# fx-erick/uncertainty-vit

Hardware: AMD Instinct MI355X
Metric: pretrain images/sec (ViT-B/16 224, bs=128/GPU) (higher is better)
Workload: dtype bf16

## Files before the change

### include/uvit.h

```cpp
#ifndef UVIT_H
#define UVIT_H
#include <stddef.h>
#include <stdint.h>

#ifdef __cplusplus
extern "C" {
#endif

#define UVIT_VERSION 100
#define UVIT_MAX_DEPTH 64

typedef struct uvit_engine uvit_engine;
typedef void* uvit_stream;

typedef struct uvit_config {
    int32_t img_size, patch_size, in_chans, embed_dim, depth, num_heads, mlp_hidden;
    int32_t use_shared_rel_pos_bias;
    int32_t use_abs_pos_emb;
    int32_t batch;
    float ln_eps;
    float attn_drop_rate;
    float drop_path_rate;
    int32_t bias_chunk;
    int32_t two_stream;
// ... 75 lines not shown
int uvit_step_backward_layer(uvit_engine* e, int layer, const uvit_step_params* hp, uvit_stream stream);
int uvit_step_wait_layer_grads(uvit_engine* e, int layer, uvit_stream stream);
int uvit_step_backward_embed(uvit_engine* e, uvit_stream stream);
int uvit_step_update(uvit_engine* e, const uvit_step_params* hp, uvit_stream stream);
int uvit_train_step(uvit_engine* e, const float* images, const int64_t* mask, const uvit_step_params* hp,
                    uvit_stream stream);
typedef struct uvit_tuning { int32_t nt_variant, tn_variant, tn_split_target, wgrad_group_chunks, nt_group, nt_persist; } uvit_tuning;
void uvit_tuning_default(uvit_tuning* out);
int uvit_engine_set_tuning(uvit_engine* e, const uvit_tuning* t);
int uvit_engine_set_streams(uvit_engine* e, int dual);
int uvit_engine_set_drop_path_rows(uvit_engine* e, int on);
int uvit_drop_path_kept_counts(int depth, float drop_path_rate, int draws_per_block, int batch, uint32_t seed, uint32_t it, int32_t* out);
int uvit_engine_profile(uvit_engine* e, int enable, int max_launches);
int uvit_engine_profile_read(uvit_engine* e, double* total_ms, int* launches, double* flops_per_launch);
int uvit_engine_profile_read_kind(uvit_engine* e, int kind, double* total_ms, int* launches, double* flops_per_launch,
                                  double* bytes_per_launch);
int uvit_engine_read_stats_async(uvit_engine* e, float* host_out2, uvit_stream stream);
int uvit_engine_read_stats(uvit_engine* e, float* host_out2, uvit_stream stream);

typedef struct uvit_gemm_epilogue {
    void* out; void* out2; const float* bias; const float* bias2; const float* gamma; const float* resid;
    const float* rowscale; const void* aux; const int64_t* mask; const float* mask_token;
    int32_t ldo, tokens, patches;
    int32_t row0;
} uvit_gemm_epilogue;
enum { UVIT_EPI_BF16 = 0, UVIT_EPI_QKV = 1, UVIT_EPI_GELU = 2, UVIT_EPI_RESID = 3, UVIT_EPI_F32 = 4,
       UVIT_EPI_PATCH = 5, UVIT_EPI_DGELU = 6, UVIT_EPI_QKV_ELU = 7,
       UVIT_EPI_GELU_DG = 8,
       UVIT_EPI_MULAUX = 9 };

int uvit_op_gemm_nt(int mode, const void* A_bf16, const void* W_bf16, int M, int N, int K, int lda, int ldw,
                    const uvit_gemm_epilogue* epi, uvit_stream stream);
int uvit_op_gemm_nt_tuned(int mode, const void* A_bf16, const void* W_bf16, int M, int N, int K, int lda, int ldw,
                          const uvit_gemm_epilogue* epi, const uvit_tuning* tune, int* tail_rows, uvit_stream stream);
typedef struct uvit_gemm_nt_plan_info { int32_t kernel, rows, grid, tail_rows; } uvit_gemm_nt_plan_info;
int uvit_op_gemm_nt_plan(int mode, int M, int N, int K, int lda, int ldw, int ldo, int row_list,
                         const uvit_tuning* tuning, int num_cu, uvit_gemm_nt_plan_info* out);
int uvit_op_gemm_nt_sched(int mode, const void* A_bf16, const void* W_bf16, int M, int N, int K, int lda, int ldw,
                          const uvit_gemm_epilogue* epi, const uvit_tuning* tune, uint32_t* tile_counters, uvit_stream stream);
int uvit_op_gemm_tn(const void* Y_bf16, const void* X_bf16, int M, int N, int K, int ldy, int ldx, float* C, int ldc,
                    const uvit_tuning* tune, uvit_stream stream);
typedef struct uvit_wgrad_problem {
    const void* Y_bf16; const void* X_bf16; float* C; float* bias; float* bias2;
    int32_t bias_end, bias2_begin, M, N, K, ldy, ldx, ldc;
} uvit_wgrad_problem;
int uvit_op_wgrad_group(const uvit_wgrad_problem* problems, int count, const uvit_tuning* tune, uvit_stream stream);
int uvit_op_attn_fwd(const void* qkv, const float* biasP, void* out, float* lse, int B, int H, int N, int NP,
                     float scale, float p_drop, uint32_t seed, uint32_t layer, uvit_stream stream);
int64_t uvit_op_attn_bwd_ws_bytes(int B, int H, int N);
int uvit_op_attn_bwd(const void* qkv, const void* o_fwd, const void* d_o, const float* biasP, const float* lse,
                           float* delta, void* dqkv, float* dbias_slab, int accumulate_slab, void* ds_workspace, int B, int H,
                           int N, int NP, float scale, float p_drop, uint32_t seed, uint32_t layer, uvit_stream stream);
int uvit_op_attn_fwd_hd(const void* qkv, const float* biasP, void* out, float* lse, int B, int H, int N, int NP, int head_dim,
                        float scale, float p_drop, uint32_t seed, uint32_t layer, uvit_stream stream);
int uvit_op_attn_bwd_hd(const void* qkv, const void* o_fwd, const void* d_o, const float* biasP, const float* lse,
                        float* delta, void* dqkv, float* dbias_slab, int accumulate_slab, void* ds_workspace, int B, int H,
                        int N, int NP, int head_dim, float scale, float p_drop, uint32_t seed, uint32_t layer, uvit_stream stream);
int uvit_op_attn2_fwd(const void* qkv_m, const void* qkv_c, const float* biasP, void* out_m, void* out_c, float* lse, int B, int H,
                      int N, int NP, float scale, float p_drop, uint32_t seed, uint32_t layer, uvit_stream stream);
int64_t uvit_op_attn2_bwd_ws_bytes(int B, int H, int N);
int uvit_op_attn2_bwd(const void* qkv_m, const void* qkv_c, const void* o_m, const void* o_c, const void* d_m, const void* d_c,
                      const float* biasP, const float* lse, float* delta, void* dqkv_m, void* dqkv_c, float* dbias_slab,
                      int accumulate_slab, void* ds_workspace, int B, int H, int N, int NP, float scale, float p_drop, uint32_t seed,
                      uint32_t layer, uvit_stream stream);
int uvit_op_relpos_gather(const float* table, const int32_t* index, float* biasP, int H, int N, int NP, uvit_stream stream);
int uvit_op_relpos_scatter(const float* slab, int nslab, const int32_t* index, float* dtable, int H, int N, int NP,
                           uvit_stream stream);
int uvit_op_ln_fwd(const float* x, const float* w, const float* b, void* y_bf16, float* mean, float* rstd, int M, int C,
                   float eps, uvit_stream stream);
int uvit_op_ln_bwd(const void* dy_bf16, const float* x, const float* mean, const float* rstd, const float* w,
                   const float* dres, float* dx, float* dw, float* db, int M, int C, uvit_stream stream);
int uvit_op_ln_fwd_walk(const float* x, const float* w, const float* b, void* y_bf16, float* mean, float* rstd, int M, int C,
                        float eps, const int32_t* rowidx, const int32_t* count, const int32_t* pos, float* xcopy, int tokens,
                        uvit_stream stream);
typedef struct uvit_ls_rider {
    const void* y; const float* gamma; const float* rowscale; void* dy; float* dgamma; float* dbias;
    int32_t tokens; const int32_t* pos; const int32_t* cnt; int32_t pad_base; void* pad2; int32_t pad2_cols;
} uvit_ls_rider;
int uvit_op_ln_bwd_walk(const void* dy_bf16, const float* x, const float* mean, const float* rstd, const float* w, const float* dres,
                        float* dx, float* dw, float* db, int M, int C, int nrep, int64_t rep_stride, const int32_t* rowidx,
                        const int32_t* count, const int32_t* pos, const uvit_ls_rider* next, uvit_stream stream);
int uvit_op_ls_bwd(const float* dx, const uvit_ls_rider* rider, int M, int C, int nrep, int64_t rep_stride, const int32_t* rowidx,
                   const int32_t* count, uvit_stream stream);
int uvit_op_colsum(const void* y_bf16, int ld, int col0, int ncols, int M, float* out, int nrep, int64_t rep_stride, uvit_stream stream);
int uvit_op_reduce_replicas(const float* rep, float* out, int64_t n, int nrep, int64_t stride, uvit_stream stream);
int uvit_op_droppath_lists(const float* scales, int32_t* pos, int32_t* bmap, int32_t* rows, int32_t* cnt, int nlists, int B, int tokens,
                           int rows_stride, const int32_t* host_counts, uvit_stream stream);
int uvit_op_gemm_nt_rows(int mode, const void* A_bf16, const void* W_bf16, int M, int N, int K, int lda, int ldw,
                         const uvit_gemm_epilogue* epi, const int32_t* rowmap, const int32_t* rowcount, const uvit_tuning* tune,
                         uvit_stream stream);
typedef struct uvit_wgrad_split { float* bias_s1; float* bias2_s1; int32_t s1_row; } uvit_wgrad_split;
int uvit_op_wgrad_group_split(const uvit_wgrad_problem* problems, const uvit_wgrad_split* split, int count, const uvit_tuning* tune,
                              uvit_stream stream);
int uvit_op_token_bwd(const float* dx, const int64_t* mask, void* dpatch_bf16, float* dcls, float* dmask_token, int B, int P, int C,
                      uvit_stream stream);
typedef struct uvit_transpose_desc { const void* src; void* dst; int32_t rows, cols, tile0, pad; } uvit_transpose_desc;
int uvit_op_transpose_batch(const uvit_transpose_desc* descs_dev, int ndesc, int total_tiles, uvit_stream stream);
int uvit_op_ema(float* ema, const float* params, void* ema_bf16, int64_t n, float decay, uvit_stream stream);
int uvit_op_sumsq(const float* g, int64_t n, double* out, uvit_stream stream);
int uvit_op_adamw(float* p, const float* g, float* m, float* v, void* p_bf16, int64_t n, int64_t n_decay, float lr,
                  float wd, float b1, float b2, float eps, int step, const double* sumsq, float max_norm,
                  float grad_scale, float* gnorm_out, uvit_stream stream);
int uvit_op_smooth_l1(const float* out, const float* target, const int32_t* count_dev, float beta, int l2,
                      float loss_scale, float* loss, void* dout_bf16, int Mmax, int C, uvit_stream stream);
int uvit_op_wasserstein_loss(const float* out_m, const float* out_c, const float* tgt_m, const float* tgt_c,
                             const int32_t* count_dev, float lam, float loss_scale, float* scratch, float* loss,
                             void* dout_m_bf16, void* dout_c_bf16, int Mmax, int C, uvit_stream stream);
int uvit_op_target_accum(const float* x, const int32_t* rowidx, const int32_t* count, float* acc, int first, int Mmax,
                         int C, float eps, uvit_stream stream);
int uvit_op_variance_loss(const float* out, const int32_t* count_dev, float w, float margin, float loss_scale, float* scratch,
                          float* loss, float* std_loss0_out, void* dout_bf16, int Mmax, int C, uvit_stream stream);
int uvit_op_target_finalize(float* acc, const int32_t* count, int n_layers, int post_ln, int Mmax, int C, float eps,
                            uvit_stream stream);
int uvit_op_mask_compact(const int64_t* mask, int32_t* rowidx, int32_t* count, int B, int P, uvit_stream stream);
int uvit_op_synth_batch(float* images, int64_t* mask, int B, int chans, int img_size, int patches, int n_mask, uint32_t seed,
                        uint32_t it, uvit_stream stream);
int uvit_op_im2col(const float* img, void* cols_bf16, int B, int Cin, int img_size, int patch, uvit_stream stream);
int uvit_op_droppath(float* scales, const float* rates_dev, int depth, int B, uint32_t seed, uint32_t step,
                     uvit_stream stream);
int uvit_op_cast_bf16(const float* src, void* dst_bf16, int64_t n, uvit_stream stream);

#define UVIT_AUG_LANCZOS 1
#define UVIT_AUG_BILINEAR 2
#define UVIT_AUG_BICUBIC 3
#define UVIT_AUG_HAMMING 5
#define UVIT_AUG_BRIGHTNESS 0
#define UVIT_AUG_CONTRAST 1
#define UVIT_AUG_SATURATION 2
typedef struct uvit_augment_desc {
    int64_t offset;
    int32_t h, w;
    int32_t flip;
    int32_t crop_x, crop_y, crop_w, crop_h;
    int32_t resize_w, resize_h;
    int32_t win_x, win_y;
    int32_t filter;
    int32_t n_jitter;
    int32_t jitter_op[3];
    float jitter_factor[3];
    int32_t reserved;
} uvit_augment_desc;
int64_t uvit_op_augment_ws_bytes(const uvit_augment_desc* desc, int B, int S);
int uvit_op_augment_batch(const uint8_t* pixels, int64_t pixel_bytes, const uvit_augment_desc* desc, int B, int S, const float* mean,
                          const float* std, float* out, void* workspace, int64_t ws_bytes, uvit_stream stream);

int64_t uvit_op_probe_pool_ws_bytes(int B, int N, int C);
int uvit_op_probe_pool_norm(const float* x, float* feat, float* scratch, int B, int N, int C, float eps, uvit_stream stream);
int uvit_op_probe_logits(const float* feat, const float* W, const float* bias, float* logits, int B, int K, int C, uvit_stream stream);
int uvit_op_probe_ce(const float* logits, const int64_t* labels, float smoothing, float* dlogits, float* row_loss, float* loss_out,
                     int32_t* top1_top5, int B, int K, uvit_stream stream);
int uvit_op_probe_head_grad(const float* dlogits, const float* feat, float* dW, float* dbias, int B, int K, int C, uvit_stream stream);

int uvit_op_calib_softmax(const float* logits, float* probs, int B, int K, uvit_stream stream);
int uvit_op_calib_confidence(const float* probs, const int64_t* labels, const double* bounds, int n_bins, int positional_acc, float* row_conf,
                             int32_t* row_pred_correct, double* row_nll, double* bin_table, double* ece_nll, int B, int K,
                             uvit_stream stream);
int uvit_op_calib_tace(const float* probs, const int64_t* labels, double threshold, int n_bins, int positional_acc, double* per_class,
                       double* tace, int B, int K, uvit_stream stream);
int uvit_op_calib_auroc(const float* probs, const int64_t* labels, int32_t* rows, double* out, int B, int K, uvit_stream stream);

int uvit_op_stability_ranks(const float* logits, int32_t* ranks, int R, int K, uvit_stream stream);
int uvit_op_stability_sequences(const int32_t* ranks, double* seq, int V, int F, int K, int noise, uvit_stream stream);

int uvit_op_gp_features(const float* feat, const float* gamma, const float* beta, const float* W_rf, const float* b_rf, float scale,
                        float ln_eps, float* ghat, float* u, float* phi, int B, int C, int D, uvit_stream stream);
int uvit_op_gp_precision_update(const float* phi, float* P, int B, int D, double momentum, uvit_stream stream);
// ... 82 lines not shown
```

### uncertainty-vit_amd/csrc/elementwise.hip

```cpp
#include "common.h"
#include "uvit_internal.h"
#include "rowwise.h"

__global__ void im2col_kernel(const float* __restrict__ img, bf16* __restrict__ cols, int B, int Cin, int S, int p) {
    const int g = S / p, P = g * g, K = Cin * p * p, kc_per_row = K / 8;
    const size_t total = (size_t)B * P * kc_per_row;
    for (size_t idx = blockIdx.x * (size_t)blockDim.x + threadIdx.x; idx < total; idx += (size_t)gridDim.x * blockDim.x) {
        const int kc = idx % kc_per_row;
        const size_t row = idx / kc_per_row;
        const int b = row / P, pp = row % P, py = pp / g, px = pp % g;
        const int k = kc * 8, c = k / (p * p), i = (k % (p * p)) / p, j = k % p;
        const float* src = img + (((size_t)b * Cin + c) * S + py * p + i) * S + px * p + j;
        const float4 a = *(const float4*)src, d = *(const float4*)(src + 4);
        bf16x8 o = {f2bf(a.x), f2bf(a.y), f2bf(a.z), f2bf(a.w), f2bf(d.x), f2bf(d.y), f2bf(d.z), f2bf(d.w)};
        *(bf16x8*)(cols + row * K + k) = o;
    }
}

__global__ __launch_bounds__(1024)
void mask_compact_kernel(const int64_t* __restrict__ mask, int* __restrict__ rowidx, int* __restrict__ count, int B, int P) {
    __shared__ int s_w[16];
    const int n = B * P, tid = threadIdx.x, lane = tid & 63, wave = tid >> 6;
    int base = 0;
    for (int sc = 0; sc < n; sc += 32 * 1024) {
        unsigned bits = 0;
#pragma unroll
        for (int k = 0; k < 32; ++k) {
            const int i = sc + k * 1024 + tid;
            if (i < n && mask[i] != 0) bits |= 1u << k;
        }
        for (int k = 0; k < 32 && sc + k * 1024 < n; ++k) {
            const bool keep = (bits >> k) & 1u;
            const unsigned long long bal = __ballot(keep);
            if (lane == 0) s_w[wave] = __popcll(bal);
            __syncthreads();
            int before = base, tot = 0;
#pragma unroll
            for (int q = 0; q < 16; ++q) { const int v = s_w[q]; tot += v; if (q < wave) before += v; }
            if (keep) {
                const int i = sc + k * 1024 + tid, b = i / P;
                rowidx[before + __popcll(bal & ((1ull << lane) - 1ull))] = b * (P + 1) + 1 + (i - b * P);
            }
            base += tot;
            __syncthreads();
        }
    }
    if (tid == 0) *count = base;
    for (int i = base + tid; i < n; i += 1024) rowidx[i] = 0;
}

__global__ void set_cls_kernel(float* __restrict__ x, const float* __restrict__ cls, int B, int N, int C) {
    const int i = blockIdx.x * blockDim.x + threadIdx.x;
    if (i < B * C) { const int b = i / C, c = i - b * C; x[(size_t)b * N * C + c] = cls[c]; }
}

__global__ void relpos_gather_kernel(const float* __restrict__ table, const int* __restrict__ index,
                                     float* __restrict__ biasP, int H, int N, int NP) {
    const size_t total = (size_t)H * NP * NP;
    for (size_t i = blockIdx.x * (size_t)blockDim.x + threadIdx.x; i < total; i += (size_t)gridDim.x * blockDim.x) {
        const int k = i % NP, q = (i / NP) % NP, h = i / ((size_t)NP * NP);
        float v = 0.f;
        if (k >= N) v = -1e30f;
        else if (q < N && table) v = table[(size_t)index[q * N + k] * H + h] * 1.4426950408889634f;
        biasP[i] = v;
    }
}

__global__ void relpos_scatter_kernel(const float* __restrict__ slab, int nslab, const int* __restrict__ index,
                                      float* __restrict__ dtable, int H, int N, int NP, int ntable) {
    extern __shared__ float tsum[];
    const int h = blockIdx.x;
    for (int i = threadIdx.x; i < ntable; i += blockDim.x) tsum[i] = 0.f;
    __syncthreads();
    const int total = N * N;
    for (int i = blockIdx.y * blockDim.x + threadIdx.x; i < total; i += gridDim.y * blockDim.x) {
        const int k = i / N, q = i - k * N;
        float s = 0.f;
        for (int sl = 0; sl < nslab; ++sl) s += slab[(((size_t)sl * H + h) * NP + k) * NP + q];
        atomicAdd(&tsum[index[q * N + k]], s);
    }
    __syncthreads();
    for (int i = threadIdx.x; i < ntable; i += blockDim.x)
        if (tsum[i] != 0.f) atomicAdd(dtable + (size_t)i * H + h, tsum[i]);
}

#define CP_ROWS 32

template <int NV, int WAVES = 4>
__device__ __forceinline__ void block_col_atomic(float4 (&acc)[NV], float* out, int nv, float (*red)[64 * 4]) {
    const int lane = threadIdx.x & 63, wave = threadIdx.x >> 6;
#pragma unroll
    for (int k = 0; k < NV; ++k) {
        if (64 * k < nv) {
            __syncthreads();
            ((float4*)red[wave])[lane] = acc[k];
            __syncthreads();
            if (wave == 0) {
                float4 s = ((float4*)red[0])[lane];
#pragma unroll
                for (int q = 1; q < WAVES; ++q) { const float4 a = ((float4*)red[q])[lane]; s.x += a.x; s.y += a.y; s.z += a.z; s.w += a.w; }
                const int i = lane + 64 * k;
                if (i < nv) { atomicAdd(out + 4 * i, s.x); atomicAdd(out + 4 * i + 1, s.y); atomicAdd(out + 4 * i + 2, s.z); atomicAdd(out + 4 * i + 3, s.w); }
            }
        }
    }
}

template <int NV>
__global__ __launch_bounds__(256)
void ls_bwd_kernel(const float* __restrict__ dx, const bf16* __restrict__ y, const float* __restrict__ gamma,
                   const float* __restrict__ rowscale, bf16* __restrict__ dy, float* __restrict__ dgamma,
                   float* __restrict__ dbias, int M, int C, int tokens, int nrep, size_t rep_stride,
                   const int* __restrict__ rowidx, const int* __restrict__ count) {
    __shared__ float red[4][64 * 4];
    dgamma += (size_t)(blockIdx.x % nrep) * rep_stride; dbias += (size_t)(blockIdx.x % nrep) * rep_stride;
    const int lane = threadIdx.x & 63, wave = threadIdx.x >> 6, nv = C >> 2;
    float4 ag[NV], ab[NV];
#pragma unroll
    for (int k = 0; k < NV; ++k) { ag[k] = make_float4(0.f, 0.f, 0.f, 0.f); ab[k] = ag[k]; }
    const int row_end = min((int)(blockIdx.x + 1) * CP_ROWS, M);
    const int n_valid = rowidx ? min(*count, M) : M;
    for (int row = blockIdx.x * CP_ROWS + wave; row < row_end; row += 4) {
        if (row >= n_valid) { store_zero_row<NV>(dy + (size_t)row * C, nv, lane); continue; }
        const int xr = rowidx ? rowidx[row] : row;
        const float dp = rowscale ? rowscale[xr / tokens] : 1.0f;
#pragma unroll
        for (int k = 0; k < NV; ++k) {
            const int i = lane + 64 * k;
            if (i < nv) {
                const float4 d = ((const float4*)(dx + (size_t)xr * C))[i];
                const float4 g = ((const float4*)gamma)[i];
                const bf16x4 yy = ((const bf16x4*)(y + (size_t)xr * C))[i];
                ls_apply(d, dp, yy, g, (bf16x4*)(dy + (size_t)row * C) + i, ag[k], ab[k]);
            }
        }
    }
    block_col_atomic(ag, dgamma, nv, red);
    block_col_atomic(ab, dbias, nv, red);
}

#define CS_ROWS 256
__global__ __launch_bounds__(256)
void colsum_kernel(const bf16* __restrict__ y, int ld, int col0, int ncols, int M, float* __restrict__ out, int nrep, size_t rep_stride) {
    __shared__ float red[4][64 * 8];
    out += (size_t)(blockIdx.y % nrep) * rep_stride;
    const int lane = threadIdx.x & 63, wave = threadIdx.x >> 6;
    const int c = blockIdx.x * 512 + lane * 8;
    float acc[8];
#pragma unroll
    for (int j = 0; j < 8; ++j) acc[j] = 0.f;
    const int row_end = min((int)(blockIdx.y + 1) * CS_ROWS, M);
    if (c < ncols) {
        const bf16* base = y + col0 + c;
        int row = blockIdx.y * CS_ROWS + wave;
        for (; row + 12 < row_end; row += 16) {
            const bf16x8 v0 = *(const bf16x8*)(base + (size_t)row * ld), v1 = *(const bf16x8*)(base + (size_t)(row + 4) * ld);
            const bf16x8 v2 = *(const bf16x8*)(base + (size_t)(row + 8) * ld), v3 = *(const bf16x8*)(base + (size_t)(row + 12) * ld);
#pragma unroll
            for (int j = 0; j < 8; ++j) acc[j] += (bf2f(v0[j]) + bf2f(v1[j])) + (bf2f(v2[j]) + bf2f(v3[j]));
        }
        for (; row < row_end; row += 4) {
            const bf16x8 v = *(const bf16x8*)(base + (size_t)row * ld);
#pragma unroll
            for (int j = 0; j < 8; ++j) acc[j] += bf2f(v[j]);
        }
    }
#pragma unroll
    for (int j = 0; j < 8; ++j) red[wave][lane * 8 + j] = acc[j];
    __syncthreads();
    for (int i = threadIdx.x; i < 512; i += 256) {
        const int cc = blockIdx.x * 512 + i;
        if (cc < ncols) atomicAdd(out + cc, red[0][i] + red[1][i] + red[2][i] + red[3][i]);
    }
}

__global__ __launch_bounds__(256)
void smooth_l1_kernel(const float* __restrict__ out, const float* __restrict__ target, const int* __restrict__ count,
                      float beta, int l2, float loss_scale, float* __restrict__ loss, bf16* __restrict__ dout,
                      int Mmax, int C) {
    __shared__ float red[4];
    const int n_valid = min(*count, Mmax);
    const size_t nv = (size_t)Mmax * C / 4, valid = (size_t)n_valid * C / 4;
    const float inv = loss_scale / ((float)n_valid * (float)C);
    float part = 0.f;
    for (size_t i = blockIdx.x * (size_t)blockDim.x + threadIdx.x; i < nv; i += (size_t)gridDim.x * blockDim.x) {
        bf16x4 g = bf16x4_zero();
        if (i < valid) {
            const float4 o = ((const float4*)out)[i], t = ((const float4*)target)[i];
            const float d[4] = {o.x - t.x, o.y - t.y, o.z - t.z, o.w - t.w};
#pragma unroll
            for (int j = 0; j < 4; ++j) {
                const float a = fabsf(d[j]);
                float l, gr;
                if (l2) { l = d[j] * d[j]; gr = 2.0f * d[j]; }
                else if (a < beta) { l = 0.5f * d[j] * d[j] / beta; gr = d[j] / beta; }
                else { l = a - 0.5f * beta; gr = d[j] > 0.f ? 1.0f : (d[j] < 0.f ? -1.0f : 0.f); }
                part += l;
                g[j] = f2bf(gr * inv);
            }
        }
        ((bf16x4*)dout)[i] = g;
    }
    part = wave_sum(part);
    if ((threadIdx.x & 63) == 0) red[threadIdx.x >> 6] = part;
    __syncthreads();
    if (threadIdx.x == 0) atomicAdd(loss, (red[0] + red[1] + red[2] + red[3]) * inv);
}

template <int NV, int TKB_WAVES>
__global__ __launch_bounds__(TKB_WAVES * 64)
void token_bwd_kernel(const float* __restrict__ dx, const int64_t* __restrict__ mask, bf16* __restrict__ dpatch,
                      float* __restrict__ dcls, float* __restrict__ dmask, int B, int P, int C, int rows_per_block) {
    __shared__ float red[TKB_WAVES][64 * 4];
    const int lane = threadIdx.x & 63, wave = threadIdx.x >> 6, nv = C >> 2, N = P + 1;
    float4 ac[NV], am[NV];
#pragma unroll
    for (int k = 0; k < NV; ++k) { ac[k] = make_float4(0.f, 0.f, 0.f, 0.f); am[k] = ac[k]; }
    const int M = B * N;
    const int row_end = min((int)(blockIdx.x + 1) * rows_per_block, M);
    for (int row = blockIdx.x * rows_per_block + wave; row < row_end; row += TKB_WAVES) {
        const int b = row / N, t = row - b * N;
// ... 72 lines not shown
        v = uvit_hash32((uint32_t)b ^ key) >= uvit_drop_threshold(r) ? 1.0f / (1.0f - r) : 0.f;
    }
    scales[i] = v;
}

#define DP_MAX_LISTS 128
struct DpHostCounts { int k[DP_MAX_LISTS]; };
#define DPL_CHUNKS 8
__global__ __launch_bounds__(256)
void droppath_lists_kernel(const float* __restrict__ scales, int* __restrict__ pos, int* __restrict__ bmap, int* __restrict__ rows,
                           int* __restrict__ cnt, int B, int tokens, int rows_stride, DpHostCounts host) {
    extern __shared__ int s_m[];
    const int lb = blockIdx.x;
    const float* sc = scales + (size_t)lb * B;
    int* p = pos + (size_t)lb * B; int* m = bmap + (size_t)lb * B; int* r = rows + (size_t)lb * rows_stride;
    const bool pub = blockIdx.y == 0;
    __shared__ int s_w[4];
    const int lane = threadIdx.x & 63, wave = threadIdx.x >> 6;
    int base = 0;
    for (int b0 = 0; b0 < B; b0 += 256) {
        const int b = b0 + threadIdx.x;
        const bool keep = b < B && sc[b] != 0.f;
        const unsigned long long bal = __ballot(keep);
        if (lane == 0) s_w[wave] = __popcll(bal);
        __syncthreads();
        int before = base;
        for (int q = 0; q < wave; ++q) before += s_w[q];
        const int slot = before + __popcll(bal & ((1ull << lane) - 1ull));
        if (pub && b < B) p[b] = keep ? slot : -1;
        if (keep) { s_m[slot] = b; if (pub) m[slot] = b; }
        base += s_w[0] + s_w[1] + s_w[2] + s_w[3];
        __syncthreads();
    }
    if (pub) {
        for (int b = base + threadIdx.x; b < B; b += 256) m[b] = 0;
        if (threadIdx.x == 0) {
            cnt[lb] = base * tokens;
            cnt[gridDim.x + lb] = base != host.k[lb];
        }
    }
    const int n = base * tokens, npad = (n + 63) & ~63;
    const int per = (npad + DPL_CHUNKS - 1) / DPL_CHUNKS, lo = blockIdx.y * per, hi = min(lo + per, npad);
    for (int i = lo + threadIdx.x; i < hi; i += blockDim.x) {
        const int slot = i / tokens;
        r[i] = i < n ? s_m[slot] * tokens + (i - slot * tokens) : -1;
    }
}

static inline int grid_for(size_t n, int block, int cap = 256 * 8) {
    size_t g = (n + block - 1) / block;
    return (int)(g < 1 ? 1 : (g > (size_t)cap ? cap : g));
}

int uvit_im2col_launch(const float* img, void* cols, int B, int Cin, int S, int p, hipStream_t s) {
    if (B <= 0 || p % 8 || S % p || S % 4) return UVIT_ERR_SHAPE;
    const size_t total = (size_t)B * (S / p) * (S / p) * (Cin * p * p / 8);
    hipLaunchKernelGGL(im2col_kernel, dim3(grid_for(total, 256, 256 * 16)), dim3(256), 0, s, img, (bf16*)cols, B, Cin, S, p);
    return uvit_check_launch();
}
int uvit_mask_compact_launch(const int64_t* mask, int* rowidx, int* count, int B, int P, hipStream_t s) {
    hipLaunchKernelGGL(mask_compact_kernel, dim3(1), dim3(1024), 0, s, mask, rowidx, count, B, P);
    return uvit_check_launch();
}
int uvit_set_cls_launch(float* x, const float* cls, const float* pos, int B, int N, int C, hipStream_t s) {
    if (pos) return UVIT_ERR_ARG;
    hipLaunchKernelGGL(set_cls_kernel, dim3((B * C + 255) / 256), dim3(256), 0, s, x, cls, B, N, C);
    return uvit_check_launch();
}
int uvit_relpos_gather_launch(const float* table, const int* index, float* biasP, int H, int N, int NP, hipStream_t s) {
    hipLaunchKernelGGL(relpos_gather_kernel, dim3(grid_for((size_t)H * NP * NP, 256)), dim3(256), 0, s, table, index, biasP, H, N, NP);
    return uvit_check_launch();
}
int uvit_relpos_scatter_launch(const float* slab, int nslab, const int* index, float* dtable, int H, int N, int NP,
                               hipStream_t s) {
    const int g = (int)(sqrtf((float)(N - 1)) + 0.5f);
    const int ntable = (2 * g - 1) * (2 * g - 1) + 3;
    hipLaunchKernelGGL(relpos_scatter_kernel, dim3(H, 24), dim3(256), ntable * sizeof(float), s, slab, nslab, index, dtable, H, N, NP, ntable);
    return uvit_check_launch();
}
int uvit_ls_bwd_launch(const float* dx, const LsNext& ls, int M, int C, int nrep, size_t rep_stride, hipStream_t s,
                       const int* rowidx, const int* count) {
    if (C % 4 || C > ROW_MAXV * 256 || (rowidx && !count)) return UVIT_ERR_SHAPE;
    dispatch_nv(C, [&](auto nv) {
        hipLaunchKernelGGL(ls_bwd_kernel<decltype(nv)::value>, dim3((M + CP_ROWS - 1) / CP_ROWS), dim3(256), 0, s, dx, ls.y, ls.gamma, ls.rowscale,
                           ls.dy, ls.dgamma, ls.dbias, M, C, ls.tokens, nrep > 0 ? nrep : 1, rep_stride, rowidx, count);
    });
    return uvit_check_launch();
}
__global__ void rows_guard_kernel(const int* __restrict__ count, int limit, float* __restrict__ loss) {
    if (*count > limit) loss[0] = __builtin_nanf("");
}
int uvit_rows_guard_launch(const int* count, int limit, float* loss, hipStream_t s) {
    hipLaunchKernelGGL(rows_guard_kernel, dim3(1), dim3(1), 0, s, count, limit, loss);
    return uvit_check_launch();
}
int uvit_colsum_launch(const void* y, int ld, int col0, int ncols, int M, float* out, int nrep, size_t rep_stride, hipStream_t s) {
    if (ncols % 8 || col0 % 8 || ld % 8) return UVIT_ERR_SHAPE;
    hipLaunchKernelGGL(colsum_kernel, dim3((ncols + 511) / 512, (M + CS_ROWS - 1) / CS_ROWS), dim3(256), 0, s, (const bf16*)y, ld, col0, ncols, M, out, nrep > 0 ? nrep : 1, rep_stride);
    return uvit_check_launch();
}
int uvit_smooth_l1_launch(const float* out, const float* target, const int* count, float beta, int l2, float loss_scale,
                          float* loss, void* dout, int Mmax, int C, hipStream_t s) {
    if (C % 4) return UVIT_ERR_SHAPE;
    hipLaunchKernelGGL(smooth_l1_kernel, dim3(grid_for((size_t)Mmax * C / 4, 256, 512)), dim3(256), 0, s, out, target, count, beta, l2,
                       loss_scale, loss, (bf16*)dout, Mmax, C);
    return uvit_check_launch();
}
int uvit_token_bwd_launch(const float* dx, const int64_t* mask, void* dpatch, float* dcls, float* dmask_token, int B,
                          int P, int C, hipStream_t s) {
    if (C % 4 || C > ROW_MAXV * 256) return UVIT_ERR_SHAPE;
    const int M = B * (P + 1);
    int rpb = (M + 127) / 128;
    rpb = ((rpb + 15) / 16) * 16;
    if (rpb < 32) rpb = 32;
    dispatch_nv(C, [&](auto nv) {
        hipLaunchKernelGGL((token_bwd_kernel<decltype(nv)::value, 16>), dim3((M + rpb - 1) / rpb), dim3(16 * 64), 0, s, dx, mask, (bf16*)dpatch,
                           dcls, dmask_token, B, P, C, rpb);
    });
    return uvit_check_launch();
}
int uvit_transpose_batch_launch(const void* descs_dev, int ndesc, int total_tiles, hipStream_t s) {
    if (ndesc <= 0 || total_tiles <= 0) return UVIT_OK;
    hipLaunchKernelGGL(transpose_batch_kernel, dim3(total_tiles), dim3(256), 0, s, (const TransposeDesc*)descs_dev, ndesc);
    return uvit_check_launch();
}
int uvit_droppath_launch(float* scales, const float* rates_dev, int depth, int nbr, int B, uint32_t seed, uint32_t step, hipStream_t s) {
    hipLaunchKernelGGL(droppath_kernel, dim3((depth * nbr * B + 255) / 256), dim3(256), 0, s, scales, rates_dev, depth, nbr, B, seed, step);
    return uvit_check_launch();
}

__global__ void droppath_lists_guard_kernel(const int* __restrict__ flags, int n, float* __restrict__ loss) {
    int bad = 0;
    for (int i = 0; i < n; ++i) bad |= flags[i];
    if (bad) loss[0] = __builtin_nanf("");
}
int uvit_droppath_lists_guard_launch(const int* cnt, int nlists, float* loss, hipStream_t s) {
    hipLaunchKernelGGL(droppath_lists_guard_kernel, dim3(1), dim3(1), 0, s, cnt + nlists, nlists, loss);
    return uvit_check_launch();
}
int uvit_droppath_lists_launch(const float* scales, int* pos, int* bmap, int* rows, int* cnt, int nlists, int B, int tokens,
                               int rows_stride, const int* host_counts, hipStream_t s) {
    if (nlists < 1 || nlists > DP_MAX_LISTS || rows_stride < ((B * tokens + 63) & ~63)) return UVIT_ERR_ARG;
    DpHostCounts h;
    for (int i = 0; i < DP_MAX_LISTS; ++i) h.k[i] = i < nlists ? host_counts[i] : 0;
    hipLaunchKernelGGL(droppath_lists_kernel, dim3(nlists, DPL_CHUNKS), dim3(256), (size_t)B * sizeof(int), s, scales, pos, bmap, rows, cnt, B, tokens, rows_stride, h);
    return uvit_check_launch();
}

__global__ void poison_kernel(const float* __restrict__ loss, float* __restrict__ dst, int* __restrict__ sticky) {
    if ((__float_as_uint(*loss) & 0x7F800000u) == 0x7F800000u) { *dst = __int_as_float(0x7FC00000); if (sticky) *sticky = 1; }
}
int uvit_poison_if_nonfinite_launch(const float* loss, float* dst, int* sticky, hipStream_t s) {
    hipLaunchKernelGGL(poison_kernel, dim3(1), dim3(1), 0, s, loss, dst, sticky);
    return uvit_check_launch();
}

__device__ __forceinline__ float sig_(float x) { return 1.0f / (1.0f + __expf(-x)); }

__global__ __launch_bounds__(256)
void wl_pos_kernel(const float* __restrict__ om, const float* __restrict__ oc, const float* __restrict__ tm,
                   const float* __restrict__ tc, const int* __restrict__ count, float* __restrict__ scratch, int Mmax, int C) {
    const int lane = threadIdx.x & 63, row = blockIdx.x * 4 + (threadIdx.x >> 6);
    if (row >= min(*count, Mmax)) return;
    float acc = 0.f;
    for (int i = lane; i < C; i += 64) {
        const size_t o = (size_t)row * C + i;
        const float d = sig_(om[o]) - sig_(tm[o]);
        const float e = sqrtf(fmaxf(sig_(oc[o]), 1e-24f)) - sqrtf(fmaxf(sig_(tc[o]), 1e-24f));
        acc += d * d + e * e;
// ... 203 lines not shown
```

### uncertainty-vit_amd/csrc/engine.hip

```cpp
#include <hip/hip_runtime.h>
#include <math.h>
#include <stdio.h>
#include <stdlib.h>
#include <string.h>

#include <string>
#include <vector>

#include "../../include/uvit.h"
#include "common.h"
#include "uvit_internal.h"

#define CHECK(x) do { int _rc = (x); if (_rc) return _rc; } while (0)
#define NREP 32
#define RP(off) (e->grep + ((off) - e->lo.n_decay))
#define HIPCHECK(x) do { if ((x) != hipSuccess) return UVIT_ERR_LAUNCH; } while (0)
#define GEMM_NT(...) uvit_gemm_nt_launch(__VA_ARGS__, &e->tune)
#define GEMM_TN(...) uvit_gemm_tn_launch(__VA_ARGS__, &e->tune)
#define GEMM_TN_GROUP(...) uvit_gemm_tn_group_launch(__VA_ARGS__, &e->tune)

struct LayerOff { size_t n1w, n1b, qkvw, qb[2], vb[2], projw[2], projb[2], g1, n2w, n2b, fc1w, fc1b, fc2w, fc2b, g2, cqkvw; };
struct Layout {
    size_t cls[2], mask_tok[2], pew[2], peb[2], relt, normw, normb, lmw[2], lmb[2], pos;
    LayerOff L[UVIT_MAX_DEPTH];
// ... 72 lines not shown
    lo.lmb[0] = add("lm_head.bias", {C}, 0);
    if (two) lo.lmb[1] = add("cov_lm_head.bias", {C}, 0);
    lo.n_live = off;
    if (two)
        for (int i = 0; i < c->depth; ++i) lo.L[i].cqkvw = add(blk(i, "attn.cov_qkv.weight"), {3 * C, C}, 2);
    lo.n_total = off;
}

struct LayerActs {
    bf16 *ln1, *qkv, *attn, *projout, *ln2, *h, *a, *mlpout;
    float *mean1, *rstd1, *mean2, *rstd2, *lse;
};

struct uvit_engine {
    uvit_config cfg;
    uvit_buffers buf;
    Layout lo;
    int B, P, N, NP, C, Hd, H, Kpe, M, Mpad, BP, BPpad;
    int head_dim;
    float attn_scale;
    int S;
    GemmTune tune;
    int cur_B;
    int tail_which = -1, tail_B = 0, tail_first = 0;
    bf16* cols;
    float* X[UVIT_MAX_DEPTH + 1];
    float* XM[UVIT_MAX_DEPTH];
    LayerActs acts[UVIT_MAX_DEPTH];
    LayerActs tacts;
    float *tX[2], *tXM;
    int *rowidx, *count;
    bf16 *normed[2], *dout[2], *dnormed[2], *dpatch[2];
    float *meanF[2], *rstdF[2], *outputs[2], *targets[2];
    float *biasP_s, *biasP_t, *slabs, *delta;
    void* ds_ws[2] = {nullptr, nullptr};
    float *dXa, *dXb;
    bf16 *dY1[2], *dY2[2], *dH[2], *dLN, *dAttn, *dqkv[2];
    float *dp_scales, *dp_rates;
    int *dpl_pos = nullptr, *dpl_bmap = nullptr, *dpl_rows = nullptr, *dpl_cnt = nullptr;
    size_t dpl_stride = 0;
    int dpl_K[128] = {};
    bool dpl_enable = true;
    bool dpl_on = false;
    std::vector<float> dp_rates_host;
    float *loss, *gnorm; double* sumsq;
    float* wl_scratch;
    float *dense_v, *dense_acc; int *idrows, *idcount;
    float* var_scratch;
    int* poisoned;
    TransposeDesc* tdesc; int n_tdesc, n_ttiles;
    int64_t* mask_copy;
    unsigned* tile_cnt = nullptr;
    float* grep;
    size_t n_nd;
    bool slab_started;
    bool last_dropout; uint32_t last_seed;
    int bwd_next = -1;
    int compact_R = 0;
    bool dual = true;
    hipStream_t aux = nullptr, aux_eq = nullptr, aux_lo = nullptr;
    hipEvent_t ev_fork = nullptr, ev_teacher = nullptr, ev_x = nullptr;
    hipEvent_t ev_wdone[UVIT_MAX_DEPTH] = {};
    hipEvent_t ev_ds = nullptr;
    bool prof_on = false;
    std::vector<hipEvent_t> prof_ev;
    std::vector<int> prof_kind;
    std::vector<int> prof_rows;
    size_t prof_used = 0;
    size_t rows_all() const { return (size_t)(S - 1) * Mpad + M; }
    size_t rows_alloc() const { return (size_t)S * Mpad; }
};

struct Bump {
    char* base; size_t off, cap;
    template <typename T> T* take(size_t n) {
        off = (off + 255) & ~(size_t)255;
        T* p = base ? (T*)(base + off) : nullptr;
        off += n * sizeof(T);
        return p;
    }
};

static size_t roundup(size_t x, size_t m) { return (x + m - 1) / m * m; }
static std::vector<float> dp_rates_linspace(int depth, float rate);

static void plan_workspace(uvit_engine* e, Bump& b) {
    const uvit_config& c = e->cfg;
    const size_t Mp = e->rows_alloc(), C = e->C, Hd = e->Hd, BPp = e->BPpad;
    auto acts = [&](LayerActs& a) {
        a.ln1 = b.take<bf16>(Mp * C); a.qkv = b.take<bf16>(Mp * 3 * C); a.attn = b.take<bf16>(Mp * C);
        a.projout = b.take<bf16>(Mp * C); a.ln2 = b.take<bf16>(Mp * C); a.h = b.take<bf16>(Mp * Hd);
        a.a = b.take<bf16>(Mp * Hd); a.mlpout = b.take<bf16>(Mp * C);
        a.mean1 = b.take<float>(Mp); a.rstd1 = b.take<float>(Mp); a.mean2 = b.take<float>(Mp); a.rstd2 = b.take<float>(Mp);
        a.lse = b.take<float>((size_t)e->B * e->H * e->N);
    };
    e->cols = b.take<bf16>(BPp * e->Kpe);
    for (int i = 0; i <= c.depth; ++i) e->X[i] = b.take<float>(Mp * C);
    for (int i = 0; i < c.depth; ++i) { e->XM[i] = b.take<float>(Mp * C); acts(e->acts[i]); }
    acts(e->tacts);
    e->tX[0] = b.take<float>(Mp * C); e->tX[1] = b.take<float>(Mp * C); e->tXM = b.take<float>(Mp * C);
    e->rowidx = b.take<int>(e->BP + 64); e->count = b.take<int>(64);
    for (int st = 0; st < e->S; ++st) {
        e->normed[st] = b.take<bf16>(BPp * C); e->dout[st] = b.take<bf16>(BPp * C); e->dnormed[st] = b.take<bf16>(BPp * C);
        e->dpatch[st] = b.take<bf16>(BPp * C);
        e->meanF[st] = b.take<float>(BPp); e->rstdF[st] = b.take<float>(BPp);
        e->outputs[st] = b.take<float>(BPp * C); e->targets[st] = b.take<float>(BPp * C);
    }
    const size_t bias_n = (size_t)e->H * e->NP * e->NP;
    e->biasP_s = b.take<float>(bias_n); e->biasP_t = b.take<float>(bias_n);
    e->slabs = b.take<float>(bias_n);
    e->delta = b.take<float>((size_t)e->B * e->H * e->N);
    if (e->cfg.use_shared_rel_pos_bias)
        for (int k = 0; k < 2; ++k)
            e->ds_ws[k] = b.take<char>(e->S == 1 ? uvit_attn_bwd_fused_ws_bytes(e->B, e->H, e->N) : uvit_attn2_bwd_ws_bytes(e->B, e->H, e->N));
    e->dXa = b.take<float>(Mp * C); e->dXb = b.take<float>(Mp * C);
    for (int k = 0; k < 2; ++k) {
        e->dY1[k] = b.take<bf16>(Mp * C); e->dY2[k] = b.take<bf16>(Mp * C); e->dH[k] = b.take<bf16>(Mp * Hd);
        e->dqkv[k] = b.take<bf16>(Mp * 3 * C);
    }
    e->dLN = b.take<bf16>(Mp * C); e->dAttn = b.take<bf16>(Mp * C);
    e->dp_scales = b.take<float>((size_t)c.depth * 2 * e->S * e->B); e->dp_rates = b.take<float>(c.depth);
    if ((size_t)c.depth * 2 * e->S <= 128) {
        const size_t nl = (size_t)c.depth * 2 * e->S;
        e->dpl_stride = roundup((size_t)e->B * e->N, 64);
        e->dpl_pos = b.take<int>(nl * e->B); e->dpl_bmap = b.take<int>(nl * e->B);
        e->dpl_rows = b.take<int>(nl * e->dpl_stride); e->dpl_cnt = b.take<int>(2 * nl + 64);
    }
    e->loss = b.take<float>(64); e->gnorm = e->loss + 1; e->sumsq = (double*)(e->loss + 2);
    e->wl_scratch = b.take<float>(16 + BPp);
    e->poisoned = b.take<int>(64);
    e->var_scratch = b.take<float>(2 * C + 16);
    e->dense_v = b.take<float>(BPp * C); e->dense_acc = b.take<float>(BPp * C);
    e->idrows = b.take<int>(e->BP + 64); e->idcount = b.take<int>(64);
    e->tdesc = b.take<TransposeDesc>(7 * c.depth + 4);
    e->mask_copy = b.take<int64_t>(e->BP + 64);
    e->grep = b.take<float>((size_t)NREP * e->n_nd);
    e->tile_cnt = b.take<unsigned>(64);
}

static void fill_dims(uvit_engine* e) {
    const uvit_config& c = e->cfg;
    const int g = c.img_size / c.patch_size;
    e->B = c.batch; e->P = g * g; e->N = e->P + 1; e->NP = 208; e->C = c.embed_dim; e->Hd = c.mlp_hidden;
    e->H = c.num_heads; e->Kpe = c.in_chans * c.patch_size * c.patch_size;
    e->head_dim = c.embed_dim / c.num_heads;
    e->attn_scale = e->head_dim == 64 ? 0.125f : (float)(1.0 / std::sqrt((double)e->head_dim));
    e->S = c.two_stream ? 2 : 1;
    e->M = e->B * e->N; e->Mpad = (int)roundup(e->M, 128); e->BP = e->B * e->P; e->BPpad = (int)roundup(e->BP, 128);
    e->cur_B = e->B;
    Layout tmp_lo; build_layout(&e->cfg, tmp_lo);
    e->n_nd = tmp_lo.n_live - tmp_lo.n_decay;
}

extern "C" void uvit_engine_destroy(uvit_engine* e);
extern "C" int uvit_version(void) { return UVIT_VERSION; }
#ifndef UVIT_SRC_HASH
#define UVIT_SRC_HASH "unknown"
#endif
extern "C" const char* uvit_source_hash(void) { return UVIT_SRC_HASH; }

extern "C" int uvit_layout_count(const uvit_config* cfg) {
    if (cfg_ok(cfg)) return UVIT_ERR_SHAPE;
    Layout lo; build_layout(cfg, lo);
    return (int)lo.entries.size();
}
extern "C" int uvit_layout_get(const uvit_config* cfg, int index, uvit_layout_entry* out) {
// ... 237 lines not shown
    bool any = false;
    for (int i = 0; i < nbr * depth; ++i) {
        const int K = e->dpl_K[i], br = i % nbr;
        any = any || (K > 0 && K < Bc && (e->S == 1 || (br & 1)));
    }
    e->dpl_on = any;
    if (!any) return UVIT_OK;
    return uvit_droppath_lists_launch(e->dp_scales, e->dpl_pos, e->dpl_bmap, e->dpl_rows, e->dpl_cnt, nbr * depth, Bc, e->N,
                                      (int)e->dpl_stride, e->dpl_K, s);
}

enum RowMode { ROWS_ALL, ROWS_LIST, ROWS_LIST2, ROWS_MASKED };
enum Pass { PASS_DENSE, PASS_TEACHER, PASS_STUDENT };
struct BranchRows {
    RowMode mode = ROWS_ALL;
    int K = 0;
    int n[2] = {0, 0};
    size_t off[2] = {0, 0};
    int rows = 0;
    int red = 0;
    DpList d[2] = {};
    const int* rowmap[2] = {nullptr, nullptr};
    const int* rowcnt[2] = {nullptr, nullptr};
};
static BranchRows branch_rows(const uvit_engine* e, int l, int branch, Pass pass, int Bc) {
    const int S = e->S;
    BranchRows r;
    r.K = Bc; r.n[0] = r.n[1] = Bc * e->N; r.off[1] = e->Mpad;
    if (pass != PASS_DENSE && branch == 1 && l == e->cfg.depth - 1 && e->compact_R > 0) {
        r.mode = ROWS_MASKED; r.n[0] = e->compact_R; r.rowmap[0] = e->rowidx; r.rowcnt[0] = e->count;
    } else if (pass == PASS_STUDENT && e->dpl_on && (S == 1 || branch == 1)) {
        DpList d[2] = {};
        bool none = false, some = false;
        for (int st = 0; st < S; ++st) {
            dp_list_get(e, l, st, branch, d[st]);
            none = none || d[st].K == 0; some = some || d[st].K < e->B;
        }
        if (!none && some) {
            r.mode = S == 1 ? ROWS_LIST : ROWS_LIST2;
            r.K = d[0].K;
            for (int st = 0; st < S; ++st) { r.d[st] = d[st]; r.n[st] = d[st].K * e->N; r.rowmap[st] = d[st].rows; r.rowcnt[st] = d[st].cnt; }
            r.off[1] = r.n[0];
        }
    }
    r.rows = (int)(r.off[S - 1] + r.n[S - 1]);
    r.red = (int)roundup(r.rows, 64);
    return r;
}

struct Draw { bool on; uint32_t seed, it; };
struct FwdPass {
    Pass kind;
    Pass rows;
    int which;
    Weights w;
    float* biasP;
    unsigned* tile_cnt;
    Draw draw;
    bool dp_on; float pdrop;
    uint32_t aseed;
    int Bc; hipStream_t s;
    const uvit_step_params* hp;
    bool dense;
};
static FwdPass fwd_pass(uvit_engine* e, Pass kind, int which, int Bc, Draw draw, const uvit_step_params* hp, hipStream_t s) {
    FwdPass p;
    p.kind = kind; p.which = which; p.w = weights_of(e, which); p.biasP = which ? e->biasP_t : e->biasP_s;
    p.tile_cnt = e->tile_cnt + (kind == PASS_TEACHER ? 16 : 0);
    const bool train = draw.on && !which;
    p.dp_on = train && e->cfg.drop_path_rate > 0.f; p.pdrop = train ? e->cfg.attn_drop_rate : 0.f;
    p.aseed = uvit_hash32(draw.seed ^ (draw.it * 0x85EBCA6Bu + 0x1234567u));
    p.draw = draw; p.Bc = Bc; p.s = s; p.hp = hp;
    p.dense = hp && (hp->target_batch_norm || hp->target_instance_norm || hp->post_target_instance_norm || !hp->target_layer_norm_last);
    p.rows = p.dense ? PASS_DENSE : kind;
    return p;
}

static int forward_layer(uvit_engine* e, const FwdPass& p, int l, const float* x_in, float* x_mid, float* x_out, LayerActs& a) {
    const LayerOff& o = e->lo.L[l];
    const Weights& w = p.w; hipStream_t s = p.s;
    const int Bc = p.Bc, M = Bc * e->N, C = e->C, Hd = e->Hd, S = e->S;
    const size_t Mp = e->Mpad;
    const bool save = p.kind == PASS_STUDENT;
    const BranchRows at = branch_rows(e, l, 0, p.rows, Bc), ml = branch_rows(e, l, 1, p.rows, Bc);
    LnFwd n1; n1.x = x_in; n1.w = w.f + o.n1w; n1.b = w.f + o.n1b; n1.y = a.ln1; n1.mean = a.mean1; n1.rstd = a.rstd1; n1.M = at.rows; n1.C = C;
    n1.eps = e->cfg.ln_eps;
    if (at.mode == ROWS_LIST) { n1.pos = at.d[0].pos; n1.xcopy = x_mid; n1.tokens = e->N; n1.M = M; }
    CHECK(uvit_ln_fwd_launch(n1, s));
    for (int st = 0; st < S; ++st) {
        GemmEpi q; q.out = a.qkv + at.off[st] * 3 * C; q.bias = w.f + o.qb[st]; q.bias2 = w.f + o.vb[st]; q.ldo = 3 * C;
        q.tile_counter = p.tile_cnt;
        CHECK(GEMM_NT(st ? EPI_QKV_ELU : EPI_QKV, a.ln1 + at.off[st] * C, w.b + o.qkvw, at.n[st], 3 * C, C, C, C, &q, s));
    }
    if (S == 1) {
        CHECK(uvit_attn_fwd_launch(a.qkv, p.biasP, a.attn, a.lse, at.K, e->H, e->N, e->NP, e->attn_scale, p.pdrop, p.aseed, (uint32_t)l, s, at.d[0].bmap,
                                   e->head_dim));
    } else {
        CHECK(uvit_attn2_fwd_launch(a.qkv, a.qkv + Mp * 3 * C, p.biasP, a.attn, a.attn + Mp * C, a.lse, Bc, e->H, e->N, e->NP, 0.125f,
                                    p.pdrop, p.aseed, (uint32_t)l, s));
    }
    auto prof_begin = [&](int kind, int rows) -> bool {
        if (!(e->prof_on && e->prof_used + 2 <= e->prof_ev.size())) return false;
        e->prof_kind[e->prof_used / 2] = kind; e->prof_rows[e->prof_used / 2] = rows;
        (void)hipEventRecord(e->prof_ev[e->prof_used], s);
        return true;
    };
    auto prof_end = [&](bool on) { if (on) { (void)hipEventRecord(e->prof_ev[e->prof_used + 1], s); e->prof_used += 2; } };
    for (int st = 0; st < S; ++st) {
        GemmEpi pj; pj.out = x_mid + st * Mp * C; pj.out2 = save ? a.projout + st * Mp * C : nullptr; pj.bias = w.f + o.projb[st];
        pj.gamma = w.f + o.g1; pj.resid = x_in + st * Mp * C; pj.rowscale = dp_ptr(e, p.dp_on, l, st, 0, Bc); pj.ldo = C; pj.tokens = e->N;
        pj.rowmap = at.rowmap[st]; pj.rowcount = at.rowcnt[st];
        const bool pp = prof_begin(UVIT_PROF_PROJ, at.n[st]);
        CHECK(GEMM_NT(EPI_RESID, a.attn + at.off[st] * C, w.b + o.projw[st], at.n[st], C, C, C, C, &pj, s));
        prof_end(pp);
    }
    LnFwd n2; n2.x = x_mid; n2.w = w.f + o.n2w; n2.b = w.f + o.n2b; n2.y = a.ln2; n2.mean = a.mean2; n2.rstd = a.rstd2; n2.M = ml.rows; n2.C = C;
    n2.eps = e->cfg.ln_eps;
    if (ml.mode == ROWS_LIST || ml.mode == ROWS_LIST2) {
        n2.tokens = e->N; n2.M = M;
        for (int st = 0; st < S; ++st) {
            n2.x = x_mid + st * Mp * C; n2.pos = ml.d[st].pos; n2.xcopy = x_out + st * Mp * C;
            n2.y = a.ln2 + ml.off[st] * C; n2.mean = a.mean2 + ml.off[st]; n2.rstd = a.rstd2 + ml.off[st];
            CHECK(uvit_ln_fwd_launch(n2, s));
        }
    } else {
        n2.rowidx = ml.rowmap[0]; n2.count = ml.rowcnt[0];
        CHECK(uvit_ln_fwd_launch(n2, s));
    }
    GemmEpi f1; f1.out = a.a; f1.out2 = save ? a.h : nullptr; f1.bias = w.f + o.fc1b; f1.ldo = Hd; f1.tile_counter = p.tile_cnt;
    const bool prof = prof_begin(save ? UVIT_PROF_FC1_S : UVIT_PROF_FC1_T, ml.rows);
    CHECK(GEMM_NT(save ? EPI_GELU_DG : EPI_GELU, a.ln2, w.b + o.fc1w, ml.rows, Hd, C, C, C, &f1, s));
    prof_end(prof);
    for (int st = 0; st < S; ++st) {
        GemmEpi f2; f2.out = x_out + st * Mp * C; f2.out2 = save ? a.mlpout + st * Mp * C : nullptr; f2.bias = w.f + o.fc2b;
        f2.gamma = w.f + o.g2; f2.resid = x_mid + st * Mp * C; f2.rowscale = dp_ptr(e, p.dp_on, l, st, 1, Bc); f2.ldo = C; f2.tokens = e->N;
        f2.rowmap = ml.rowmap[st]; f2.rowcount = ml.rowcnt[st];
        const bool pf2 = prof_begin(UVIT_PROF_FC2, ml.n[st]);
        CHECK(GEMM_NT(EPI_RESID, a.a + ml.off[st] * Hd, w.b + o.fc2w, ml.n[st], C, Hd, Hd, Hd, &f2, s));
        prof_end(pf2);
    }
    return UVIT_OK;
}

static int embed(uvit_engine* e, const Weights& w, const int64_t* mask, float* x0, int Bc, hipStream_t s) {
    for (int st = 0; st < e->S; ++st) {
        float* x = x0 + (size_t)st * e->Mpad * e->C;
        GemmEpi pe; pe.out = x; pe.bias = w.f + e->lo.peb[st]; pe.mask = mask; pe.mask_token = w.f + e->lo.mask_tok[st]; pe.ldo = e->C; pe.patches = e->P;
        CHECK(GEMM_NT(EPI_PATCH, e->cols, w.b + e->lo.pew[st], Bc * e->P, e->C, e->Kpe, e->Kpe, e->Kpe, &pe, s));
        CHECK(uvit_set_cls_launch(x, w.f + e->lo.cls[st], nullptr, Bc, e->N, e->C, s));
        if (e->cfg.use_abs_pos_emb) CHECK(uvit_add_pos_launch(x, w.f + e->lo.pos, Bc, e->N, e->C, s));
    }
    return UVIT_OK;
}

struct TargetBuild { bool dense; int n; };
static int targets_after_layer(uvit_engine* e, const FwdPass& p, TargetBuild& t, int l, const float* xout) {
    const uvit_step_params* hp = p.hp; const int Bc = p.Bc; hipStream_t s = p.s;
    if (t.dense && Bc != e->B) return UVIT_ERR_ARG;
    for (int k = 0; k < hp->n_target_layers; ++k) {
        if (hp->target_layers[k] != l) continue;
        const float* sub = hp->layer_results_fc ? e->tXM : nullptr;
        for (int st = t.dense ? 1 : 0; st < e->S; ++st)
            CHECK(uvit_target_accum_launch(xout + (size_t)st * e->Mpad * e->C, e->rowidx, e->count, e->targets[st], t.n == 0,
                                           Bc * e->P, e->C, 1e-5f, s, sub ? sub + (size_t)st * e->Mpad * e->C : nullptr,
                                           hp->target_layer_norm_last ? 1 : 0));
        if (t.dense) {
            CHECK(uvit_gather_patch_rows_launch(xout, sub, e->dense_v, Bc, e->P, e->C, s));
            if (hp->target_batch_norm) CHECK(uvit_colnorm_launch(e->dense_v, 1, Bc * e->P, e->C, 1e-5f, s));
            if (hp->target_instance_norm) CHECK(uvit_colnorm_launch(e->dense_v, Bc, e->P, e->C, 1e-5f, s));
            if (hp->target_layer_norm_last)
                CHECK(uvit_target_accum_launch(e->dense_v, e->idrows, e->idcount, e->dense_acc, t.n == 0, Bc * e->P, e->C, 1e-5f, s));
            else CHECK(uvit_axpy_rows_launch(e->dense_acc, e->dense_v, t.n == 0, (size_t)Bc * e->P * e->C, s));
        }
        ++t.n;
    }
    return UVIT_OK;
}
static int targets_finalize(uvit_engine* e, const FwdPass& p, const TargetBuild& t) {
    const uvit_step_params* hp = p.hp; const int Bc = p.Bc; hipStream_t s = p.s;
    if (t.n != hp->n_target_layers) return UVIT_ERR_ARG;
    for (int st = t.dense ? 1 : 0; st < e->S; ++st)
        CHECK(uvit_target_finalize_launch(e->targets[st], e->count, t.n, hp->post_target_layer_norm, Bc * e->P, e->C, 1e-5f, s));
    if (t.dense) {
        const bool pin = hp->post_target_instance_norm != 0;
        CHECK(uvit_target_finalize_launch(e->dense_acc, e->idcount, t.n, hp->post_target_layer_norm && !pin, Bc * e->P, e->C, 1e-5f, s));
        if (pin) {
            CHECK(uvit_colnorm_launch(e->dense_acc, Bc, e->P, e->C, 1e-5f, s));
            if (hp->post_target_layer_norm)
                CHECK(uvit_target_finalize_launch(e->dense_acc, e->idcount, 1, 1, Bc * e->P, e->C, 1e-5f, s));
        }
        CHECK(uvit_gather_masked_rows_launch(e->dense_acc, e->rowidx, e->count, e->targets[0], Bc * e->P, e->P, e->C, s));
    }
    return UVIT_OK;
}

static int run_forward(uvit_engine* e, const FwdPass& p, const float* images, const int64_t* mask) {
    const int Bc = p.Bc; hipStream_t s = p.s;
    if (Bc < 1 || Bc > e->B) return UVIT_ERR_SHAPE;
    if (p.kind == PASS_DENSE) CHECK(uvit_im2col_launch(images, e->cols, Bc, e->cfg.in_chans, e->cfg.img_size, e->cfg.patch_size, s));
    CHECK(uvit_relpos_gather_launch(e->cfg.use_shared_rel_pos_bias ? p.w.f + e->lo.relt : nullptr, e->buf.rel_index, p.biasP,
                                    e->H, e->N, e->NP, s));
    if (p.dp_on) CHECK(uvit_droppath_launch(e->dp_scales, e->dp_rates, e->cfg.depth, 2 * e->S, Bc, p.draw.seed, p.draw.it, s));
    if (!p.which) {
        e->dpl_on = false;
        if (p.dp_on && p.kind == PASS_STUDENT && e->dpl_enable && Bc == e->B) CHECK(dp_lists_begin(e, p.draw.seed, p.draw.it, Bc, s));
        e->last_dropout = p.draw.on; e->last_seed = p.aseed;
    }
    const bool keep = p.kind != PASS_TEACHER;
    CHECK(embed(e, p.w, mask, keep ? e->X[0] : e->tX[0], Bc, s));
    TargetBuild tb{p.dense, 0};
    for (int l = 0; l < e->cfg.depth; ++l) {
        float* xout = keep ? e->X[l + 1] : e->tX[(l + 1) & 1];
        CHECK(forward_layer(e, p, l, keep ? e->X[l] : e->tX[l & 1], keep ? e->XM[l] : e->tXM, xout, keep ? e->acts[l] : e->tacts));
        if (!keep) CHECK(targets_after_layer(e, p, tb, l, xout));
    }
    if (!keep) CHECK(targets_finalize(e, p, tb));
    e->cur_B = Bc;
// ... 115 lines not shown
    if (e->S == 1 && hp->n_rows_hint > 0) {
        const int R = (int)roundup((size_t)(hp->n_rows_hint < BP ? hp->n_rows_hint : BP), 64);
        if (R >= 512 && R < e->M) {
            e->compact_R = R;
            CHECK(uvit_zero_launch(e->dXb, e->rows_alloc() * C * sizeof(float), ts));
            CHECK(uvit_zero_launch(e->dY2[(e->cfg.depth - 1) & 1], e->rows_alloc() * C * sizeof(bf16), ts));
        }
    }
    HIPCHECK(hipMemcpyAsync(e->mask_copy, mask, (size_t)BP * sizeof(int64_t), hipMemcpyDeviceToDevice, s));
    CHECK(uvit_mask_compact_launch(mask, e->rowidx, e->count, Bc, e->P, s));
    CHECK(uvit_im2col_launch(images, e->cols, Bc, e->cfg.in_chans, e->cfg.img_size, e->cfg.patch_size, s));
    if (e->dual) { HIPCHECK(hipEventRecord(e->ev_fork, s)); HIPCHECK(hipStreamWaitEvent(ts, e->ev_fork, 0)); }
    const FwdPass teacher = fwd_pass(e, PASS_TEACHER, 1, Bc, Draw{false, 0, 0}, hp, ts);
    const FwdPass student = fwd_pass(e, PASS_STUDENT, 0, Bc, Draw{hp->train_dropout != 0, hp->seed, hp->it}, nullptr, s);
    CHECK(run_forward(e, teacher, images, nullptr));
    if (e->dual) HIPCHECK(hipEventRecord(e->ev_teacher, ts));
    CHECK(run_forward(e, student, images, mask));
    const int Rh = e->compact_R > 0 ? e->compact_R : BP;
    for (int st = 0; st < e->S; ++st) CHECK(head_forward(e, student.w, Bc, st, false, e->outputs[st], s, e->compact_R));
    if (e->dual) HIPCHECK(hipStreamWaitEvent(s, e->ev_teacher, 0));
    const float ls = hp->loss_scale == -1.0f ? 1.0f : hp->loss_scale;
    CHECK(uvit_smooth_l1_launch(e->outputs[0], e->targets[0], e->count, hp->l1_beta, hp->l2_loss, ls, e->loss, e->dout[0], BP, C, s));
    if (hp->var_w0 > 0.f)
        CHECK(uvit_variance_loss_launch(e->outputs[0], e->count, hp->var_w0, hp->var_margin0, ls, e->var_scratch, e->loss, e->loss + 4,
                                        e->dout[0], BP, C, s));
    if (e->compact_R > 0) CHECK(uvit_rows_guard_launch(e->count, e->compact_R, e->loss, s));
    if (e->dpl_on) CHECK(uvit_droppath_lists_guard_launch(e->dpl_cnt, 2 * e->S * e->cfg.depth, e->loss, s));
    if (e->S == 2)
        CHECK(uvit_wasserstein_loss_launch(e->outputs[0], e->outputs[1], e->targets[0], e->targets[1], e->count, hp->lambda_pretraining,
                                           ls, e->wl_scratch, e->loss, e->dout[0], e->dout[1], BP, C, s));
    float* g = e->buf.grads;
    const bf16* wt = (const bf16*)e->buf.params_bf16_t;
    for (int st = 0; st < e->S; ++st) {
        const size_t lmw = lo.lmw[st], lmb = lo.lmb[st];
        TnProb hw; hw.Y = e->dout[st]; hw.X = e->normed[st]; hw.C = g + lmw; hw.M = e->compact_R > 0 ? e->compact_R : e->BPpad; hw.Nn = C; hw.Kk = C;
        hw.ldy = C; hw.ldx = C; hw.ldc = C; hw.bias = RP(lmb); hw.bias_end = C;
        CHECK(wgrad(e, &hw, 1, s));
        GemmEpi d; d.out = e->dnormed[st]; d.ldo = C;
        CHECK(GEMM_NT(EPI_BF16, e->dout[st], wt + lmw, Rh, C, C, C, C, &d, s));
        LnBwd fn; fn.dy = e->dnormed[st]; fn.x = e->X[e->cfg.depth] + (size_t)st * e->Mpad * C; fn.rowidx = e->rowidx; fn.count = e->count;
        fn.mean = e->meanF[st]; fn.rstd = e->rstdF[st]; fn.w = e->buf.params + lo.normw; fn.dx = e->dXa + (size_t)st * e->Mpad * C;
        fn.dw = RP(lo.normw); fn.db = RP(lo.normb); fn.M = Rh; fn.C = C; fn.nrep = NREP; fn.rep_stride = e->n_nd;
        CHECK(uvit_ln_bwd_launch(fn, s));
    }
    return UVIT_OK;
}

extern "C" int uvit_step_backward_layer(uvit_engine* e, int l, const uvit_step_params* hp, uvit_stream stream) {
    if (!e || l < 0 || l >= e->cfg.depth || l != e->bwd_next) return UVIT_ERR_ARG;
    (void)hp;
    e->bwd_next = l - 1;
    hipStream_t s = (hipStream_t)stream;
    const LayerOff& o = e->lo.L[l];
    LayerActs& a = e->acts[l];
    const int M = e->M, C = e->C, Hd = e->Hd, S = e->S;
    const size_t Mp = e->Mpad;
    float* g = e->buf.grads;
    const float* pf = e->buf.params;
    const bf16* wt = (const bf16*)e->buf.params_bf16_t;
    const bool dp_on = e->last_dropout && e->cfg.drop_path_rate > 0.f;
    const float pdrop = e->last_dropout ? e->cfg.attn_drop_rate : 0.f;
    const int par = l & 1;
    hipStream_t ws = e->dual ? e->aux : s;
    if (e->dual && l + 2 < e->cfg.depth) HIPCHECK(hipStreamWaitEvent(s, e->ev_wdone[l + 2], 0));
    bf16 *dY1 = e->dY1[par], *dY2 = e->dY2[par], *dH = e->dH[par], *dqkv = e->dqkv[par];
    const BranchRows at = branch_rows(e, l, 0, PASS_STUDENT, e->B), ml = branch_rows(e, l, 1, PASS_STUDENT, e->B);
    const BranchRows nx = l > 0 ? branch_rows(e, l - 1, 1, PASS_STUDENT, e->B) : BranchRows{};
    const int Mmlp = ml.mode == ROWS_ALL ? ml.rows : ml.red;
    if (S == 2 && ml.mode == ROWS_ALL && Mp > (size_t)M) CHECK(uvit_zero_launch(dY1 + (size_t)M * C, (Mp - M) * C * sizeof(bf16), s));
    TnProb wg[UVIT_TN_GROUP_MAX];
    int nwg = 0;
    {
        TnProb& f2 = wg[nwg++]; f2.Y = dY1; f2.X = a.a; f2.C = g + o.fc2w; f2.M = ml.red; f2.Nn = C; f2.Kk = Hd; f2.ldy = C; f2.ldx = Hd; f2.ldc = Hd;
        TnProb& f1 = wg[nwg++]; f1.Y = dH; f1.X = a.ln2; f1.C = g + o.fc1w; f1.M = ml.red; f1.Nn = Hd; f1.Kk = C; f1.ldy = Hd; f1.ldx = C; f1.ldc = C;
        f1.bias = RP(o.fc1b); f1.bias_end = Hd;
        for (int st = 0; st < S; ++st) {
            TnProb& pj = wg[nwg++]; pj.Y = dY2 + at.off[st] * C; pj.X = a.attn + at.off[st] * C; pj.C = g + o.projw[st];
            pj.M = (int)roundup(at.n[st], 64); pj.Nn = C; pj.Kk = C; pj.ldy = C; pj.ldx = C; pj.ldc = C;
        }
        TnProb& qk = wg[nwg++]; qk.Y = dqkv; qk.X = a.ln1; qk.C = g + o.qkvw; qk.M = at.red; qk.Nn = 3 * C; qk.Kk = C; qk.ldy = 3 * C; qk.ldx = C; qk.ldc = C;
        qk.bias = RP(o.qb[0]); qk.bias_end = C; qk.bias2 = RP(o.vb[0]); qk.bias2_begin = 2 * C;
        if (S == 2) { qk.bias_s1 = RP(o.qb[1]); qk.bias2_s1 = RP(o.vb[1]); qk.s1_row = (int)Mp; }
    }
    auto mlp_rider = [&](int layer, int st, const BranchRows& br, bf16* dY) {
        const LayerOff& L = e->lo.L[layer];
        LsNext n; n.y = e->acts[layer].mlpout + st * Mp * C; n.gamma = pf + L.g2; n.rowscale = dp_ptr(e, dp_on, layer, st, 1, e->B);
        n.dy = dY + br.off[st] * C; n.dgamma = RP(L.g2); n.dbias = RP(L.fc2b); n.tokens = e->N;
        return n;
    };
    if (l == e->cfg.depth - 1)
        for (int st = 0; st < S; ++st)
            CHECK(uvit_ls_bwd_launch(e->dXa + st * Mp * C, mlp_rider(l, st, ml, dY1), (ml.mode == ROWS_ALL || st + 1 < S) ? ml.n[st] : ml.red - (int)ml.off[st],
                                     C, NREP, e->n_nd, s, ml.rowmap[st], ml.rowcnt[st]));
    GemmEpi d1; d1.out = dH; d1.aux = a.h; d1.ldo = Hd;
    CHECK(GEMM_NT(EPI_MULAUX, dY1, wt + o.fc2w, Mmlp, Hd, C, C, C, &d1, s));
    GemmEpi d2; d2.out = e->dLN; d2.ldo = C;
    CHECK(GEMM_NT(EPI_BF16, dH, wt + o.fc1w, Mmlp, C, Hd, Hd, Hd, &d2, s));
    const bool ln2_samples = ml.mode != ROWS_MASKED && (ml.mode != ROWS_ALL || at.mode == ROWS_LIST);
    for (int st = 0; st < S; ++st) {
        const size_t eo = st * Mp * C;
        LnBwd b; b.dy = e->dLN + ml.off[st] * C; b.x = e->XM[l] + eo; b.mean = a.mean2 + ml.off[st]; b.rstd = a.rstd2 + ml.off[st]; b.w = pf + o.n2w;
        b.dres = e->dXa + eo; b.dx = e->dXb + eo; b.dw = RP(o.n2w); b.db = RP(o.n2b); b.C = C; b.nrep = NREP; b.rep_stride = e->n_nd;
        LsNext& n = b.next;
        n.y = a.projout + eo; n.gamma = pf + o.g1; n.rowscale = dp_ptr(e, dp_on, l, st, 0, e->B); n.dy = dY2 + at.off[st] * C;
        n.dgamma = RP(o.g1); n.dbias = RP(o.projb[st]); n.tokens = e->N; n.pos = at.d[st].pos;
        if (ln2_samples) { b.M = M; b.pos = ml.d[st].pos; n.cnt = at.d[st].cnt; if (at.mode == ROWS_LIST) { n.pad2 = dqkv; n.pad2_cols = 3 * C; } }
        else { b.M = ml.n[st]; b.rowidx = ml.rowmap[st]; b.count = ml.rowcnt[st]; }
        CHECK(uvit_ln_bwd_launch(b, s));
    }
    for (int st = 0; st < S; ++st) {
        GemmEpi d3; d3.out = e->dAttn + at.off[st] * C; d3.ldo = C;
        CHECK(GEMM_NT(EPI_BF16, dY2 + at.off[st] * C, wt + o.projw[st], at.n[st], C, C, C, C, &d3, s));
    }
    const float* biasP = e->biasP_s;
    float* slabs = e->cfg.use_shared_rel_pos_bias ? e->slabs : nullptr;
    {
        void* dsw = slabs ? e->ds_ws[par] : nullptr;
        if (S == 1) {
            if (at.mode == ROWS_LIST && ml.mode == ROWS_MASKED && at.red > at.rows)
                CHECK(uvit_zero_launch(dqkv + (size_t)at.rows * 3 * C, (size_t)(at.red - at.rows) * 3 * C * sizeof(bf16), s));
            CHECK(uvit_attn_bwd_fused_launch(a.qkv, a.attn, e->dAttn, biasP, a.lse, e->delta, dqkv, dsw, dsw != nullptr, at.K, e->H,
                                             e->N, e->NP, e->attn_scale, pdrop, e->last_seed, (uint32_t)l, s, at.d[0].bmap, e->head_dim));
        } else {
            CHECK(uvit_attn2_bwd_launch(a.qkv, a.qkv + Mp * 3 * C, a.attn, a.attn + Mp * C, e->dAttn, e->dAttn + Mp * C, biasP, a.lse,
                                        e->delta, dqkv, dqkv + Mp * 3 * C, dsw, dsw != nullptr, e->B, e->H, e->N, e->NP, 0.125f, pdrop,
                                        e->last_seed, (uint32_t)l, s));
        }
        if (dsw) {
            if (e->dual) { HIPCHECK(hipEventRecord(e->ev_ds, s)); HIPCHECK(hipStreamWaitEvent(ws, e->ev_ds, 0)); }
            if (S == 1) CHECK(uvit_attn_dbias_reduce_launch(dsw, slabs, e->slab_started ? 1 : 0, at.K, e->H, e->N, e->NP, ws));
            else CHECK(uvit_attn2_dbias_reduce_launch(dsw, slabs, e->slab_started ? 1 : 0, e->B, e->H, e->N, e->NP, ws));
        }
    }
    e->slab_started = true;
    if (e->dual) { HIPCHECK(hipEventRecord(e->ev_x, s)); HIPCHECK(hipStreamWaitEvent(ws, e->ev_x, 0)); }
    CHECK(wgrad(e, wg, nwg, ws));
    if (e->dual) HIPCHECK(hipEventRecord(e->ev_wdone[l], ws));
    GemmEpi d4; d4.out = e->dLN; d4.ldo = C;
    CHECK(GEMM_NT(EPI_BF16, dqkv, wt + o.qkvw, at.rows, C, 3 * C, 3 * C, 3 * C, &d4, s));
    if (l > 0 && e->dual && l + 1 < e->cfg.depth) HIPCHECK(hipStreamWaitEvent(s, e->ev_wdone[l + 1], 0));
    const bool ln1_samples = at.mode == ROWS_LIST || nx.mode != ROWS_ALL;
    for (int st = 0; st < (l > 0 ? S : 1); ++st) {
        const size_t ro = st * Mp, eo = ro * C;
        LnBwd b; b.dy = e->dLN + eo; b.x = e->X[l] + eo; b.mean = a.mean1 + ro; b.rstd = a.rstd1 + ro; b.w = pf + o.n1w; b.dres = e->dXb + eo;
        b.dx = e->dXa + eo; b.dw = RP(o.n1w); b.db = RP(o.n1b); b.M = l > 0 ? M : (int)e->rows_all(); b.C = C; b.nrep = NREP;
        b.rep_stride = e->n_nd;
        if (ln1_samples) { b.pos = at.d[st].pos; b.next.tokens = e->N; }
        if (l > 0) {
            b.next = mlp_rider(l - 1, st, nx, e->dY1[(l - 1) & 1]);
            b.next.pos = nx.d[st].pos;
            if (st + 1 == S && nx.d[st].cnt) { b.next.cnt = nx.d[st].cnt; b.next.pad_base = (int)nx.off[st]; }
        }
        CHECK(uvit_ln_bwd_launch(b, s));
    }
    return UVIT_OK;
}

extern "C" int uvit_step_backward_embed(uvit_engine* e, uvit_stream stream) {
    if (!e) return UVIT_ERR_ARG;
    hipStream_t s = (hipStream_t)stream;
    Layout& lo = e->lo;
    float* g = e->buf.grads;
    const int C = e->C, BP = e->BP;
    TnProb pe[2];
    for (int st = 0; st < e->S; ++st) {
        CHECK(uvit_token_bwd_launch(e->dXa + (size_t)st * e->Mpad * C, e->mask_copy, e->dpatch[st], g + lo.cls[st], g + lo.mask_tok[st], e->B, e->P, C, s));
        TnProb& q = pe[st]; q.Y = e->dpatch[st]; q.X = e->cols; q.C = g + lo.pew[st]; q.M = (int)roundup(BP, 64); q.Nn = C; q.Kk = e->Kpe;
        q.ldy = C; q.ldx = e->Kpe; q.ldc = e->Kpe; q.bias = RP(lo.peb[st]); q.bias_end = C;
    }
    CHECK(wgrad(e, pe, e->S, s));
    if (e->cfg.use_abs_pos_emb) CHECK(uvit_pos_bwd_launch(e->dXa, g + lo.pos, e->B, e->N, C, s));
    if (e->dual) HIPCHECK(hipStreamWaitEvent(s, e->ev_wdone[0], 0));
    if (e->cfg.use_shared_rel_pos_bias && e->slab_started)
        CHECK(uvit_relpos_scatter_launch(e->slabs, 1, e->buf.rel_index, g + lo.relt, e->H, e->N, e->NP, s));
    CHECK(uvit_reduce_replicas_launch(e->grep, g + lo.n_decay, e->n_nd, NREP, e->n_nd, s));
    CHECK(uvit_poison_if_nonfinite_launch(e->loss, g + lo.n_decay, e->poisoned, s));
    return UVIT_OK;
}

extern "C" int uvit_step_wait_layer_grads(uvit_engine* e, int layer, uvit_stream stream) {
    if (!e || layer < 0 || layer >= e->cfg.depth) return UVIT_ERR_ARG;
    if (e->dual) HIPCHECK(hipStreamWaitEvent((hipStream_t)stream, e->ev_wdone[layer], 0));
    return UVIT_OK;
}

extern "C" int uvit_step_update(uvit_engine* e, const uvit_step_params* hp, uvit_stream stream) {
    if (!e || !hp) return UVIT_ERR_ARG;
    if (hp->sched_dev && (hp->sched_len < 1 || hp->sched_index < 0 || hp->sched_index >= hp->sched_len)) return UVIT_ERR_ARG;
    hipStream_t s = (hipStream_t)stream;
    Layout& lo = e->lo;
    HIPCHECK(hipMemsetAsync(e->sumsq, 0, sizeof(double), s));
    CHECK(uvit_sumsq_launch(e->buf.grads, lo.n_live, e->sumsq, s));
    const float gs = hp->grad_scale > 0.f ? hp->grad_scale : 1.0f;
    CHECK(uvit_adamw_launch(e->buf.params, e->buf.grads, e->buf.adam_m, e->buf.adam_v, e->buf.params_bf16, lo.n_live, lo.n_decay,
                            hp->lr, hp->weight_decay, hp->beta1, hp->beta2, hp->eps, hp->opt_step, e->sumsq, hp->clip_grad, gs,
                            e->gnorm, s, e->loss, (hp->do_ema || hp->sched_dev) ? e->buf.ema : nullptr, e->buf.ema_bf16, hp->ema_decay, e->poisoned,
                            hp->sched_dev, hp->sched_len, hp->sched_index));
    CHECK(uvit_transpose_batch_launch(e->tdesc, e->n_tdesc, e->n_ttiles, s));
    return UVIT_OK;
}

extern "C" int uvit_train_step(uvit_engine* e, const float* images, const int64_t* mask, const uvit_step_params* hp,
                               uvit_stream stream) {
    CHECK(uvit_step_begin(e, images, mask, hp, stream));
    for (int l = e->cfg.depth - 1; l >= 0; --l) CHECK(uvit_step_backward_layer(e, l, hp, stream));
    CHECK(uvit_step_backward_embed(e, stream));
    return uvit_step_update(e, hp, stream);
}

extern "C" int uvit_engine_read_stats_async(uvit_engine* e, float* host_out2, uvit_stream stream) {
    if (!e || !host_out2) return UVIT_ERR_ARG;
    HIPCHECK(hipMemcpyAsync(host_out2, e->loss, 8 * sizeof(float), hipMemcpyDeviceToHost, (hipStream_t)stream));
    return UVIT_OK;
}

extern "C" int uvit_engine_read_stats(uvit_engine* e, float* host_out2, uvit_stream stream) {
    if (!e || !host_out2) return UVIT_ERR_ARG;
    hipStream_t s = (hipStream_t)stream;
    HIPCHECK(hipMemcpyAsync(host_out2, e->loss, 2 * sizeof(float), hipMemcpyDeviceToHost, s));
// ... 86 lines not shown
    return UVIT_OK;
}
extern "C" int uvit_op_attn_fwd_hd(const void* qkv, const float* biasP, void* out, float* lse, int B, int H, int N, int NP, int head_dim,
                                   float scale, float p_drop, uint32_t seed, uint32_t layer, uvit_stream st) {
    if (!qkv || !out || !lse) return UVIT_ERR_ARG;
    if (head_dim != 64 && head_dim != 80) return UVIT_ERR_SHAPE;
    return uvit_attn_fwd_launch(qkv, biasP, out, lse, B, H, N, NP, scale, p_drop, seed, layer, S(st), nullptr, head_dim);
}
extern "C" int uvit_op_attn_bwd_hd(const void* qkv, const void* o_fwd, const void* d_o, const float* biasP, const float* lse,
                                   float* delta, void* dqkv, float* slab, int acc, void* ds_ws, int B, int H, int N, int NP, int head_dim,
                                   float scale, float p_drop, uint32_t seed, uint32_t layer, uvit_stream st) {
    if (!qkv || !o_fwd || !d_o || !lse || !delta || !dqkv || (slab && !ds_ws)) return UVIT_ERR_ARG;
    if (head_dim != 64 && head_dim != 80) return UVIT_ERR_SHAPE;
    CHECK(uvit_attn_bwd_fused_launch(qkv, o_fwd, d_o, biasP, lse, delta, dqkv, ds_ws, slab != nullptr, B, H, N, NP, scale, p_drop, seed, layer,
                                     S(st), nullptr, head_dim));
    if (slab) CHECK(uvit_attn_dbias_reduce_launch(ds_ws, slab, acc, B, H, N, NP, S(st)));
    return UVIT_OK;
}
extern "C" int uvit_op_attn2_fwd(const void* qkv_m, const void* qkv_c, const float* biasP, void* out_m, void* out_c, float* lse, int B,
                                 int H, int N, int NP, float scale, float p_drop, uint32_t seed, uint32_t layer, uvit_stream st) {
    if (!qkv_m || !qkv_c || !out_m || !out_c || !lse) return UVIT_ERR_ARG;
    return uvit_attn2_fwd_launch(qkv_m, qkv_c, biasP, out_m, out_c, lse, B, H, N, NP, scale, p_drop, seed, layer, S(st));
}
extern "C" int64_t uvit_op_attn2_bwd_ws_bytes(int B, int H, int N) {
    if (B <= 0 || H <= 0 || N <= 0) return UVIT_ERR_SHAPE;
    return (int64_t)uvit_attn2_bwd_ws_bytes(B, H, N);
}
extern "C" int uvit_op_attn2_bwd(const void* qkv_m, const void* qkv_c, const void* o_m, const void* o_c, const void* d_m, const void* d_c,
                                 const float* biasP, const float* lse, float* delta, void* dqkv_m, void* dqkv_c, float* slab, int acc,
                                 void* ds_ws, int B, int H, int N, int NP, float scale, float p_drop, uint32_t seed, uint32_t layer,
                                 uvit_stream st) {
    if (!qkv_m || !qkv_c || !o_m || !o_c || !d_m || !d_c || !lse || !delta || !dqkv_m || !dqkv_c || (slab && !ds_ws)) return UVIT_ERR_ARG;
    CHECK(uvit_attn2_bwd_launch(qkv_m, qkv_c, o_m, o_c, d_m, d_c, biasP, lse, delta, dqkv_m, dqkv_c, ds_ws, slab != nullptr, B, H, N, NP,
                                scale, p_drop, seed, layer, S(st)));
    if (slab) CHECK(uvit_attn2_dbias_reduce_launch(ds_ws, slab, acc, B, H, N, NP, S(st)));
    return UVIT_OK;
}
extern "C" int uvit_op_relpos_gather(const float* t, const int32_t* idx, float* biasP, int H, int N, int NP, uvit_stream st) {
    return uvit_relpos_gather_launch(t, idx, biasP, H, N, NP, S(st));
}
extern "C" int uvit_op_relpos_scatter(const float* slab, int nslab, const int32_t* idx, float* dt, int H, int N, int NP, uvit_stream st) {
    return uvit_relpos_scatter_launch(slab, nslab, idx, dt, H, N, NP, S(st));
}
extern "C" int uvit_op_ln_fwd(const float* x, const float* w, const float* b, void* y, float* mean, float* rstd, int M, int C,
                              float eps, uvit_stream st) {
    LnFwd p; p.x = x; p.w = w; p.b = b; p.y = (bf16*)y; p.mean = mean; p.rstd = rstd; p.M = M; p.C = C; p.eps = eps;
    return uvit_ln_fwd_launch(p, S(st));
}
extern "C" int uvit_op_ln_bwd(const void* dy, const float* x, const float* mean, const float* rstd, const float* w,
                              const float* dres, float* dx, float* dw, float* db, int M, int C, uvit_stream st) {
    LnBwd p; p.dy = (const bf16*)dy; p.x = x; p.mean = mean; p.rstd = rstd; p.w = w; p.dres = dres; p.dx = dx; p.dw = dw; p.db = db; p.M = M; p.C = C;
    return uvit_ln_bwd_launch(p, S(st));
}
static LsNext ls_from_abi(const uvit_ls_rider* r) {
    LsNext n;
    if (!r) return n;
    n.y = (const bf16*)r->y; n.gamma = r->gamma; n.rowscale = r->rowscale; n.dy = (bf16*)r->dy; n.dgamma = r->dgamma; n.dbias = r->dbias;
    n.tokens = r->tokens; n.pos = r->pos; n.cnt = r->cnt; n.pad_base = r->pad_base; n.pad2 = (bf16*)r->pad2; n.pad2_cols = r->pad2_cols;
    return n;
}
extern "C" int uvit_op_ln_fwd_walk(const float* x, const float* w, const float* b, void* y, float* mean, float* rstd, int M, int C, float eps,
                                   const int32_t* rowidx, const int32_t* count, const int32_t* pos, float* xcopy, int tokens, uvit_stream st) {
    if (!x || !w || !b || !y || (!mean != !rstd)) return UVIT_ERR_ARG;
    LnFwd p; p.x = x; p.w = w; p.b = b; p.y = (bf16*)y; p.mean = mean; p.rstd = rstd; p.M = M; p.C = C; p.eps = eps;
    p.rowidx = rowidx; p.count = count; p.pos = pos; p.xcopy = xcopy; p.tokens = tokens;
    return uvit_ln_fwd_launch(p, S(st));
}
extern "C" int uvit_op_ln_bwd_walk(const void* dy, const float* x, const float* mean, const float* rstd, const float* w, const float* dres,
                                   float* dx, float* dw, float* db, int M, int C, int nrep, int64_t rep_stride, const int32_t* rowidx,
                                   const int32_t* count, const int32_t* pos, const uvit_ls_rider* next, uvit_stream st) {
    if (!dy || !x || !mean || !rstd || !w || !dx || !dw || !db || nrep < 1 || rep_stride < 0) return UVIT_ERR_ARG;
    if (next && next->dy && (!next->y || !next->gamma || !next->dgamma || !next->dbias)) return UVIT_ERR_ARG;
    LnBwd p; p.dy = (const bf16*)dy; p.x = x; p.mean = mean; p.rstd = rstd; p.w = w; p.dres = dres; p.dx = dx; p.dw = dw; p.db = db;
    p.M = M; p.C = C; p.nrep = nrep; p.rep_stride = (size_t)rep_stride; p.rowidx = rowidx; p.count = count; p.pos = pos;
    p.next = ls_from_abi(next);
    return uvit_ln_bwd_launch(p, S(st));
}
extern "C" int uvit_op_ls_bwd(const float* dx, const uvit_ls_rider* r, int M, int C, int nrep, int64_t rep_stride, const int32_t* rowidx,
                              const int32_t* count, uvit_stream st) {
    if (!dx || !r || !r->y || !r->gamma || !r->dy || !r->dgamma || !r->dbias || nrep < 1 || rep_stride < 0) return UVIT_ERR_ARG;
    if (M <= 0 || C <= 0 || r->tokens <= 0) return UVIT_ERR_SHAPE;
    return uvit_ls_bwd_launch(dx, ls_from_abi(r), M, C, nrep, (size_t)rep_stride, S(st), rowidx, count);
}
extern "C" int uvit_op_colsum(const void* y, int ld, int col0, int ncols, int M, float* out, int nrep, int64_t rep_stride, uvit_stream st) {
    if (!y || !out || nrep < 1 || rep_stride < 0) return UVIT_ERR_ARG;
    if (M <= 0 || ncols <= 0 || col0 < 0 || col0 + ncols > ld) return UVIT_ERR_SHAPE;
    return uvit_colsum_launch(y, ld, col0, ncols, M, out, nrep, (size_t)rep_stride, S(st));
}
extern "C" int uvit_op_reduce_replicas(const float* rep, float* out, int64_t n, int nrep, int64_t stride, uvit_stream st) {
    if (!rep || !out || n < 0 || nrep < 0 || stride < 0) return UVIT_ERR_ARG;
    return uvit_reduce_replicas_launch(rep, out, (size_t)n, nrep, (size_t)stride, S(st));
}
extern "C" int uvit_op_droppath_lists(const float* scales, int32_t* pos, int32_t* bmap, int32_t* rows, int32_t* cnt, int nlists, int B,
                                      int tokens, int rows_stride, const int32_t* host_counts, uvit_stream st) {
    if (!scales || !pos || !bmap || !rows || !cnt || !host_counts || B < 1 || tokens < 1) return UVIT_ERR_ARG;
    return uvit_droppath_lists_launch(scales, pos, bmap, rows, cnt, nlists, B, tokens, rows_stride, host_counts, S(st));
}
extern "C" int uvit_op_gemm_nt_rows(int mode, const void* A, const void* W, int M, int N, int K, int lda, int ldw, const uvit_gemm_epilogue* ep,
                                    const int32_t* rowmap, const int32_t* rowcount, const uvit_tuning* tune, uvit_stream st) {
    if (!A || !W || !ep || !ep->out || !ep->resid || !rowmap || !rowcount || mode != UVIT_EPI_RESID) return UVIT_ERR_ARG;
    GemmTune tu;
    const int trc = tune_from_abi(tune, tu);
    if (trc) return trc;
    GemmEpi g = epi_from_abi(ep);
    g.rowmap = rowmap; g.rowcount = rowcount;
    return uvit_gemm_nt_launch(mode, A, W, M, N, K, lda, ldw, &g, S(st), &tu, nullptr);
}
extern "C" int uvit_op_wgrad_group_split(const uvit_wgrad_problem* problems, const uvit_wgrad_split* split, int count, const uvit_tuning* tune,
                                         uvit_stream st) {
    if (!problems || !split || count < 1 || count > UVIT_TN_GROUP_MAX) return UVIT_ERR_ARG;
    GemmTune tu;
    const int trc = tune_from_abi(tune, tu);
    if (trc) return trc;
    TnProb pr[UVIT_TN_GROUP_MAX];
    for (int i = 0; i < count; ++i) {
        const uvit_wgrad_problem& q = problems[i];
        if (!q.Y_bf16 || !q.X_bf16 || !q.C) return UVIT_ERR_ARG;
        pr[i].Y = q.Y_bf16; pr[i].X = q.X_bf16; pr[i].C = q.C; pr[i].bias = q.bias; pr[i].bias2 = q.bias2;
        pr[i].bias_end = q.bias_end; pr[i].bias2_begin = q.bias2_begin;
        pr[i].M = q.M; pr[i].Nn = q.N; pr[i].Kk = q.K; pr[i].ldy = q.ldy; pr[i].ldx = q.ldx; pr[i].ldc = q.ldc;
        pr[i].bias_s1 = split[i].bias_s1; pr[i].bias2_s1 = split[i].bias2_s1; pr[i].s1_row = split[i].s1_row;
    }
    return uvit_gemm_tn_group_launch(pr, count, S(st), &tu);
}
extern "C" int uvit_op_token_bwd(const float* dx, const int64_t* mask, void* dpatch, float* dcls, float* dmask_token, int B, int P, int C,
                                 uvit_stream st) {
    if (!dx || !mask || !dpatch || !dcls || !dmask_token) return UVIT_ERR_ARG;
    if (B < 1 || P < 1 || C < 1) return UVIT_ERR_SHAPE;
    return uvit_token_bwd_launch(dx, mask, dpatch, dcls, dmask_token, B, P, C, S(st));
}
static_assert(sizeof(uvit_transpose_desc) == sizeof(TransposeDesc), "uvit_transpose_desc mirrors TransposeDesc");
extern "C" int uvit_op_transpose_batch(const uvit_transpose_desc* descs_dev, int ndesc, int total_tiles, uvit_stream st) {
    if (!descs_dev || ndesc < 1 || total_tiles < 1) return UVIT_ERR_ARG;
    return uvit_transpose_batch_launch(descs_dev, ndesc, total_tiles, S(st));
}
extern "C" int uvit_op_ema(float* ema, const float* p, void* eb, int64_t n, float d, uvit_stream st) {
    return uvit_ema_launch(ema, p, eb, (size_t)n, d, S(st));
}
extern "C" int uvit_op_sumsq(const float* g, int64_t n, double* out, uvit_stream st) { return uvit_sumsq_launch(g, (size_t)n, out, S(st)); }
extern "C" int uvit_op_adamw(float* p, const float* g, float* m, float* v, void* pb, int64_t n, int64_t nd, float lr, float wd,
                             float b1, float b2, float eps, int step, const double* sumsq, float max_norm, float gs,
                             float* gn, uvit_stream st) {
    return uvit_adamw_launch(p, g, m, v, pb, (size_t)n, (size_t)nd, lr, wd, b1, b2, eps, step, sumsq, max_norm, gs, gn, S(st));
}
extern "C" int uvit_op_smooth_l1(const float* out, const float* target, const int32_t* count, float beta, int l2, float ls,
                                 float* loss, void* dout, int Mmax, int C, uvit_stream st) {
    return uvit_smooth_l1_launch(out, target, count, beta, l2, ls, loss, dout, Mmax, C, S(st));
}
extern "C" int uvit_op_wasserstein_loss(const float* om, const float* oc, const float* tm, const float* tc, const int32_t* count, float lam,
                                        float ls, float* scratch, float* loss, void* dm, void* dc, int Mmax, int C, uvit_stream st) {
    if (!om || !oc || !tm || !tc || !count || !scratch || !loss || !dm || !dc || Mmax < 1 || C < 1) return UVIT_ERR_ARG;
    return uvit_wasserstein_loss_launch(om, oc, tm, tc, count, lam, ls, scratch, loss, dm, dc, Mmax, C, S(st));
}
extern "C" int uvit_op_variance_loss(const float* out, const int32_t* count, float w, float margin, float ls, float* scratch, float* loss,
                                     float* std_out, void* dout, int Mmax, int C, uvit_stream st) {
    if (!out || !count || !scratch || !loss || !dout) return UVIT_ERR_ARG;
    return uvit_variance_loss_launch(out, count, w, margin, ls, scratch, loss, std_out, dout, Mmax, C, S(st));
}
extern "C" int uvit_op_target_accum(const float* x, const int32_t* rowidx, const int32_t* count, float* acc, int first, int Mmax,
                                    int C, float eps, uvit_stream st) {
    return uvit_target_accum_launch(x, rowidx, count, acc, first, Mmax, C, eps, S(st));
}
extern "C" int uvit_op_target_finalize(float* acc, const int32_t* count, int nl, int post_ln, int Mmax, int C, float eps, uvit_stream st) {
    return uvit_target_finalize_launch(acc, count, nl, post_ln, Mmax, C, eps, S(st));
}
extern "C" int uvit_op_mask_compact(const int64_t* mask, int32_t* rowidx, int32_t* count, int B, int P, uvit_stream st) {
// ... 15 lines not shown
```

### uncertainty-vit_amd/csrc/norm.hip

```cpp
#include "common.h"
#include "uvit_internal.h"
#include "rowwise.h"

#define LN_WAVES 4

enum LnWalk { WALK_ROWS, WALK_SAMPLES };

template <int NV, LnWalk WALK>
__global__ __launch_bounds__(LN_WAVES * 64)
void ln_fwd_kernel(const float* __restrict__ x, const int* __restrict__ rowidx, const int* __restrict__ count,
                   const int* __restrict__ pos, const float* __restrict__ w, const float* __restrict__ b, bf16* __restrict__ y,
                   float* __restrict__ mean_o, float* __restrict__ rstd_o, float* __restrict__ xcopy, int M, int C, float eps, int tokens) {
    const int lane = threadIdx.x & 63;
    const int row = blockIdx.x * LN_WAVES + (threadIdx.x >> 6);
    if (row >= M) return;
    const int nv = C >> 2;
    int src = row;
    size_t dst = row;
    if constexpr (WALK == WALK_ROWS) {
        if (row >= (count ? *count : M)) { store_zero_row<NV>(y + (size_t)row * C, nv, lane); return; }
        if (rowidx) src = rowidx[row];
    }
    RowVec<NV> r;
    load_row(r, x + (size_t)src * C, C, lane);
    if constexpr (WALK == WALK_SAMPLES) {
        const int smp = row / tokens, slot = pos[smp];
        if (slot < 0) {
#pragma unroll
            for (int k = 0; k < NV; ++k) if (lane + 64 * k < nv) ((float4*)(xcopy + (size_t)row * C))[lane + 64 * k] = r.v[k];
            return;
        }
        dst = (size_t)slot * tokens + (row - smp * tokens);
    }
    float mean, rstd;
    row_stats(r, C, lane, eps, mean, rstd);
    if (lane == 0 && (WALK == WALK_SAMPLES || mean_o)) { mean_o[dst] = mean; rstd_o[dst] = rstd; }
    normalize_store(r, mean, rstd, w, b, y + dst * C, nv, lane);
}

#define LNB_WAVES 8

template <int NV, bool LS>
struct LnbRow {
    float4 x[NV], dres[NV];
    bf16x4 dy[NV], y[LS ? NV : 1];
    float mean, rstd, dp;
    int xr;
    int ar;
    int yr;
};

template <int NV, LnWalk WALK, bool LS>
__device__ __forceinline__ void lnb_load(LnbRow<NV, LS>& r, int row, const bf16* dy, const float* x, const int* map,
                                         const float* mean_i, const float* rstd_i, const float* dres, const LsNext& ls,
                                         int C, int nv, int lane) {
    const int tokens = ls.tokens;
    r.dp = 1.0f;
    if constexpr (WALK == WALK_ROWS) {
        const int xr = map ? map[row] : row;
        r.xr = xr; r.ar = row; r.yr = xr;
        r.mean = mean_i[row]; r.rstd = rstd_i[row];
        if constexpr (LS) {
            if (ls.rowscale) r.dp = ls.rowscale[xr / tokens];
            if (ls.pos) { const int smp = xr / tokens, sl = ls.pos[smp]; r.yr = sl < 0 ? -1 : sl * tokens + (xr - smp * tokens); }
        }
    } else {
        const int smp = row / tokens, t = row - smp * tokens;
        const int sa = map ? map[smp] : smp, sb = LS ? (ls.pos ? ls.pos[smp] : smp) : -1;
        r.xr = row;
        r.ar = sa < 0 ? -1 : sa * tokens + t;
        r.yr = sb < 0 ? -1 : sb * tokens + t;
        r.mean = 0.f; r.rstd = 0.f;
        if (r.ar >= 0) { r.mean = mean_i[r.ar]; r.rstd = rstd_i[r.ar]; }
        if (r.yr >= 0 && ls.rowscale) r.dp = ls.rowscale[smp];
    }
#pragma unroll
    for (int k = 0; k < NV; ++k) {
        const int i = lane + 64 * k;
        if (i < nv) {
            if (WALK == WALK_ROWS || r.ar >= 0) {
                r.x[k] = ((const float4*)(x + (size_t)r.xr * C))[i];
                r.dy[k] = ((const bf16x4*)(dy + (size_t)r.ar * C))[i];
            }
            r.dres[k] = WALK == WALK_SAMPLES || dres ? ((const float4*)(dres + (size_t)r.xr * C))[i] : make_float4(0.f, 0.f, 0.f, 0.f);
            if constexpr (LS) if (WALK == WALK_ROWS || r.yr >= 0) r.y[k] = ((const bf16x4*)(ls.y + (size_t)r.xr * C))[i];
        }
    }
}

template <int NV>
__device__ __forceinline__ void lnb_pad_fill(const LsNext& ls, int C, int nv, int lane, int wave) {
    const int n = *ls.cnt, npad = ((ls.pad_base + n + 63) & ~63) - ls.pad_base;
    for (int r = n + wave; r < npad; r += LNB_WAVES) {
        store_zero_row<NV>(ls.dy + (size_t)r * C, nv, lane);
        if (ls.pad2) for (int c = lane * 4; c < ls.pad2_cols; c += 256) *(bf16x4*)(ls.pad2 + (size_t)r * ls.pad2_cols + c) = bf16x4_zero();
    }
}

template <int NV, LnWalk WALK, bool LS>
__global__ __launch_bounds__(LNB_WAVES * 64)
void ln_bwd_kernel(const bf16* __restrict__ dy, const float* __restrict__ x, const int* __restrict__ map ,
                   const int* __restrict__ count, const float* __restrict__ mean_i, const float* __restrict__ rstd_i,
                   const float* __restrict__ w, const float* __restrict__ dres, float* __restrict__ dx,
                   float* __restrict__ dw, float* __restrict__ db, int M, int C, int nrep, size_t rep_stride, LsNext ls,
                   int rows_per_block) {
    __shared__ float red[LNB_WAVES][64 * 4];
    const int lane = threadIdx.x & 63, wave = threadIdx.x >> 6;
    const int nv = C >> 2;
    int n_valid = M;
    if constexpr (WALK == WALK_ROWS) { if (count) n_valid = min(*count, M); }
    if constexpr (WALK == WALK_SAMPLES && LS) { if (ls.cnt && blockIdx.x == gridDim.x - 1) lnb_pad_fill<NV>(ls, C, nv, lane, wave); }
    float4 ww[NV], gm[LS ? NV : 1];
    RowVec<NV> aw, ab;
    RowVec<LS ? NV : 1> ag, ay;
#pragma unroll
    for (int k = 0; k < NV; ++k) {
        aw.v[k] = make_float4(0.f, 0.f, 0.f, 0.f); ab.v[k] = aw.v[k];
        ww[k] = lane + 64 * k < nv ? ((const float4*)w)[lane + 64 * k] : aw.v[k];
    }
#pragma unroll
    for (int k = 0; k < (LS ? NV : 1); ++k) {
        ag.v[k] = make_float4(0.f, 0.f, 0.f, 0.f); ay.v[k] = ag.v[k]; gm[k] = ag.v[k];
        if constexpr (LS) { if (lane + 64 * k < nv) gm[k] = ((const float4*)ls.gamma)[lane + 64 * k]; }
    }
    const int row_end = min((int)(blockIdx.x + 1) * rows_per_block, n_valid);
    int row = blockIdx.x * rows_per_block + wave;
    LnbRow<NV, LS> cur, nxt;
    if (row < row_end) lnb_load<NV, WALK, LS>(cur, row, dy, x, map, mean_i, rstd_i, dres, ls, C, nv, lane);
    for (; row < row_end; row += LNB_WAVES) {
        const bool more = row + LNB_WAVES < row_end;
        if (more) lnb_load<NV, WALK, LS>(nxt, row + LNB_WAVES, dy, x, map, mean_i, rstd_i, dres, ls, C, nv, lane);
        const bool own = WALK == WALK_ROWS || cur.ar >= 0;
        const float mean = cur.mean, rstd = cur.rstd;
        float4 g[NV], h[NV];
        float s1 = 0.f, s2 = 0.f;
        if (own) {
#pragma unroll
            for (int k = 0; k < NV; ++k) {
                if (lane + 64 * k < nv) {
                    const float d0 = bf2f(cur.dy[k][0]), d1 = bf2f(cur.dy[k][1]), d2 = bf2f(cur.dy[k][2]), d3 = bf2f(cur.dy[k][3]);
                    h[k] = normalize4(cur.x[k], mean, rstd);
                    aw.v[k].x += d0 * h[k].x; aw.v[k].y += d1 * h[k].y; aw.v[k].z += d2 * h[k].z; aw.v[k].w += d3 * h[k].w;
                    ab.v[k].x += d0; ab.v[k].y += d1; ab.v[k].z += d2; ab.v[k].w += d3;
                    g[k] = make_float4(d0 * ww[k].x, d1 * ww[k].y, d2 * ww[k].z, d3 * ww[k].w);
                    s1 += g[k].x + g[k].y + g[k].z + g[k].w;
                    s2 += g[k].x * h[k].x + g[k].y * h[k].y + g[k].z * h[k].z + g[k].w * h[k].w;
                } else {
                    g[k] = make_float4(0.f, 0.f, 0.f, 0.f); h[k] = g[k];
                }
            }
            s1 = wave_sum(s1) / C;
            s2 = wave_sum(s2) / C;
        }
#pragma unroll
        for (int k = 0; k < NV; ++k) {
            const int i = lane + 64 * k;
            if (i < nv) {
                float4 o = cur.dres[k];
                if (own) o = make_float4(o.x + rstd * (g[k].x - s1 - h[k].x * s2), o.y + rstd * (g[k].y - s1 - h[k].y * s2),
                                         o.z + rstd * (g[k].z - s1 - h[k].z * s2), o.w + rstd * (g[k].w - s1 - h[k].w * s2));
                ((float4*)(dx + (size_t)cur.xr * C))[i] = o;
                if constexpr (LS) if (cur.yr >= 0)
                    ls_apply(o, cur.dp, cur.y[k], gm[k], (bf16x4*)(ls.dy + (size_t)cur.yr * C) + i, ag.v[k], ay.v[k]);
            }
        }
        if (more) cur = nxt;
    }
    const size_t rep = (size_t)(blockIdx.x % nrep) * rep_stride;
    auto fold = [&](const float4& part, float* dst, int k) {
        __syncthreads();
        ((float4*)red[wave])[lane] = part;
        __syncthreads();
        if (lane < 32) {
            const int col = wave * 32 + lane;
            float sum = 0.f;
#pragma unroll
            for (int q = 0; q < LNB_WAVES; ++q) sum += red[q][col];
            const int c = 256 * k + col;
            if (c < C) atomicAdd(dst + rep + c, sum);
        }
    };
#pragma unroll
    for (int k = 0; k < NV; ++k) {
        if (64 * k < nv) {
            fold(aw.v[k], dw, k);
            fold(ab.v[k], db, k);
            if constexpr (LS) { fold(ag.v[k], ls.dgamma, k); fold(ay.v[k], ls.dbias, k); }
        }
    }
}

template <int NV>
__global__ __launch_bounds__(LN_WAVES * 64)
void target_accum_kernel(const float* __restrict__ x, const float* __restrict__ sub, const int* __restrict__ rowidx,
                         const int* __restrict__ count, float* __restrict__ acc, int first, int Mmax, int C, float eps, int ln) {
    const int lane = threadIdx.x & 63;
    const int row = blockIdx.x * LN_WAVES + (threadIdx.x >> 6);
    if (row >= Mmax) return;
    const int nv = C >> 2;
    float4* dst = (float4*)(acc + (size_t)row * C);
    if (row >= *count) {
        if (first)
#pragma unroll
            for (int k = 0; k < NV; ++k) if (lane + 64 * k < nv) dst[lane + 64 * k] = make_float4(0.f, 0.f, 0.f, 0.f);
        return;
    }
    RowVec<NV> r;
    load_row(r, x + (size_t)rowidx[row] * C, C, lane);
    if (sub) {
        RowVec<NV> q;
        load_row(q, sub + (size_t)rowidx[row] * C, C, lane);
#pragma unroll
        for (int k = 0; k < NV; ++k) { r.v[k].x -= q.v[k].x; r.v[k].y -= q.v[k].y; r.v[k].z -= q.v[k].z; r.v[k].w -= q.v[k].w; }
    }
    float mean = 0.f, rstd = 1.f;
    if (ln) row_stats(r, C, lane, eps, mean, rstd);
    normalize_store(r, mean, rstd, (float*)dst, !first, nv, lane);
}

template <int NV>
__global__ __launch_bounds__(LN_WAVES * 64)
void target_finalize_kernel(float* __restrict__ acc, const int* __restrict__ count, float inv_layers, int post_ln,
                            int Mmax, int C, float eps) {
    const int lane = threadIdx.x & 63;
    const int row = blockIdx.x * LN_WAVES + (threadIdx.x >> 6);
    if (row >= Mmax || row >= *count) return;
    const int nv = C >> 2;
    RowVec<NV> r;
    load_row(r, acc + (size_t)row * C, C, lane);
#pragma unroll
    for (int k = 0; k < NV; ++k) { r.v[k].x *= inv_layers; r.v[k].y *= inv_layers; r.v[k].z *= inv_layers; r.v[k].w *= inv_layers; }
    float mean = 0.f, rstd = 1.f;
    if (post_ln) row_stats(r, C, lane, eps, mean, rstd);
    normalize_store(r, mean, rstd, acc + (size_t)row * C, false, nv, lane);
}

#define LNB_BLOCKS_PER_CU 1
static int lnb_rows(int M, int resident_blocks_per_cu) {
    static int ncu = 0;
    if (!ncu) {
        int dev = 0; hipDeviceProp_t prop;
        ncu = (hipGetDevice(&dev) == hipSuccess && hipGetDeviceProperties(&prop, dev) == hipSuccess && prop.multiProcessorCount > 0)
                  ? prop.multiProcessorCount : 256;
    }
    const int target = ncu * resident_blocks_per_cu;
    int rows = (M + target - 1) / target;
    rows = ((rows + LNB_WAVES - 1) / LNB_WAVES) * LNB_WAVES;
    return rows < LNB_WAVES ? LNB_WAVES : rows;
}

static int ln_shape_ok(int M, int C) { return (M > 0 && C > 0 && (C % 4) == 0 && C <= ROW_MAXV * 256) ? UVIT_OK : UVIT_ERR_SHAPE; }
static dim3 ln_grid(int M) { return dim3((M + LN_WAVES - 1) / LN_WAVES); }

int uvit_ln_fwd_launch(const LnFwd& p, hipStream_t s) {
    const bool samples = p.pos || p.xcopy;
    if (ln_shape_ok(p.M, p.C) || (samples && (p.rowidx || p.count))) return UVIT_ERR_SHAPE;
    if (samples && (p.tokens <= 0 || (p.M % p.tokens) || !p.pos || !p.xcopy || !p.mean || !p.rstd)) return UVIT_ERR_SHAPE;
    dispatch_nv(p.C, [&](auto nv) {
        constexpr int NV = decltype(nv)::value;
        hipLaunchKernelGGL((samples ? ln_fwd_kernel<NV, WALK_SAMPLES> : ln_fwd_kernel<NV, WALK_ROWS>), ln_grid(p.M), dim3(LN_WAVES * 64), 0, s,
                           p.x, p.rowidx, p.count, p.pos, p.w, p.b, p.y, p.mean, p.rstd, p.xcopy, p.M, p.C, p.eps, p.tokens);
    });
    return uvit_check_launch();
}
int uvit_ln_bwd_launch(const LnBwd& p, hipStream_t s) {
    const LsNext& n = p.next;
    const bool ls = n.dy != nullptr, samples = p.pos || n.cnt || (n.pos && !p.rowidx);
    if (ln_shape_ok(p.M, p.C) || (p.rowidx && !p.count) || (samples && (p.rowidx || p.count))) return UVIT_ERR_SHAPE;
    if ((ls || samples) && n.tokens <= 0) return UVIT_ERR_SHAPE;
    if (samples && ((p.M % n.tokens) || !p.dres)) return UVIT_ERR_SHAPE;
    if (((n.pos || n.cnt) && !ls) || n.pad_base < 0 || (n.pad2 && (!n.cnt || n.pad2_cols <= 0 || (n.pad2_cols % 4)))) return UVIT_ERR_SHAPE;
    const int rpb = lnb_rows(p.M, LNB_BLOCKS_PER_CU);
    dispatch_nv(p.C, [&](auto nv) {
        constexpr int NV = decltype(nv)::value;
        auto kernel = samples ? (ls ? ln_bwd_kernel<NV, WALK_SAMPLES, true> : ln_bwd_kernel<NV, WALK_SAMPLES, false>)
                              : (ls ? ln_bwd_kernel<NV, WALK_ROWS, true> : ln_bwd_kernel<NV, WALK_ROWS, false>);
        hipLaunchKernelGGL(kernel, dim3((p.M + rpb - 1) / rpb), dim3(LNB_WAVES * 64), 0, s, p.dy, p.x, samples ? p.pos : p.rowidx, p.count,
                           p.mean, p.rstd, p.w, p.dres, p.dx, p.dw, p.db, p.M, p.C, p.nrep > 0 ? p.nrep : 1, p.rep_stride, n, rpb);
    });
    return uvit_check_launch();
}
int uvit_target_accum_launch(const float* x, const int* rowidx, const int* count, float* acc, int first, int Mmax,
                             int C, float eps, hipStream_t s, const float* sub, int ln) {
    if (ln_shape_ok(Mmax, C)) return UVIT_ERR_SHAPE;
    dispatch_nv(C, [&](auto nv) {
        hipLaunchKernelGGL(target_accum_kernel<decltype(nv)::value>, ln_grid(Mmax), dim3(LN_WAVES * 64), 0, s, x, sub, rowidx, count, acc, first,
                           Mmax, C, eps, ln);
    });
    return uvit_check_launch();
}
int uvit_target_finalize_launch(float* acc, const int* count, int n_layers, int post_ln, int Mmax, int C, float eps,
                                hipStream_t s) {
    if (ln_shape_ok(Mmax, C) || n_layers <= 0) return UVIT_ERR_SHAPE;
    dispatch_nv(C, [&](auto nv) {
        hipLaunchKernelGGL(target_finalize_kernel<decltype(nv)::value>, ln_grid(Mmax), dim3(LN_WAVES * 64), 0, s, acc, count, 1.0f / n_layers,
                           post_ln, Mmax, C, eps);
    });
    return uvit_check_launch();
}

__global__ __launch_bounds__(256)
void reduce_replicas_kernel(const float* __restrict__ rep, float* __restrict__ out, size_t n4, int nrep, size_t stride4) {
    for (size_t i = blockIdx.x * (size_t)blockDim.x + threadIdx.x; i < n4; i += (size_t)gridDim.x * blockDim.x) {
        float4 a = ((const float4*)out)[i];
        for (int r = 0; r < nrep; ++r) {
            const float4 b = ((const float4*)rep)[(size_t)r * stride4 + i];
            a.x += b.x; a.y += b.y; a.z += b.z; a.w += b.w;
        }
        ((float4*)out)[i] = a;
    }
}
int uvit_reduce_replicas_launch(const float* rep, float* out, size_t n, int nrep, size_t stride, hipStream_t s) {
    if (n % 4 || stride % 4) return UVIT_ERR_SHAPE;
    size_t g = (n / 4 + 255) / 256;
    hipLaunchKernelGGL(reduce_replicas_kernel, dim3((unsigned)(g > 1024 ? 1024 : g)), dim3(256), 0, s, rep, out, n / 4, nrep, stride / 4);
    return uvit_check_launch();
}

__global__ __launch_bounds__(256)
void gather_patch_rows_kernel(const float* __restrict__ x, const float* __restrict__ sub, float* __restrict__ v, int B, int P, int C4) {
    const size_t total = (size_t)B * P * C4;
    for (size_t i = blockIdx.x * (size_t)blockDim.x + threadIdx.x; i < total; i += (size_t)gridDim.x * blockDim.x) {
        const size_t row = i / C4; const int c = (int)(i - row * C4);
        const int b = (int)(row / P), p_ = (int)(row - (size_t)b * P);
        const size_t src = ((size_t)b * (P + 1) + 1 + p_) * C4 + c;
        float4 a = ((const float4*)x)[src];
        if (sub) { const float4 q = ((const float4*)sub)[src]; a.x -= q.x; a.y -= q.y; a.z -= q.z; a.w -= q.w; }
        ((float4*)v)[i] = a;
    }
}

__global__ __launch_bounds__(256)
void colnorm_kernel(float* __restrict__ v, int rows, int C, float eps) {
    __shared__ double red[2][4][64];
    __shared__ float stat[2][64];
    const int ch = blockIdx.x * 64 + (threadIdx.x & 63), ph = threadIdx.x >> 6;
    float* base = v + (size_t)blockIdx.y * rows * C;
    double s1 = 0.0, s2 = 0.0;
    if (ch < C)
        for (int r = ph; r < rows; r += 4) { const double a = base[(size_t)r * C + ch]; s1 += a; s2 += a * a; }
    red[0][ph][threadIdx.x & 63] = s1; red[1][ph][threadIdx.x & 63] = s2;
    __syncthreads();
    if (ph == 0) {
        const int l = threadIdx.x;
        const double a = red[0][0][l] + red[0][1][l] + red[0][2][l] + red[0][3][l];
        const double q = red[1][0][l] + red[1][1][l] + red[1][2][l] + red[1][3][l];
        const double mean = a / rows, var = q / rows - mean * mean;
        stat[0][l] = (float)mean; stat[1][l] = (float)(1.0 / sqrt((var > 0.0 ? var : 0.0) + (double)eps));
    }
    __syncthreads();
    if (ch < C) {
        const float mean = stat[0][threadIdx.x & 63], rstd = stat[1][threadIdx.x & 63];
        for (int r = ph; r < rows; r += 4) { float* q = base + (size_t)r * C + ch; *q = (*q - mean) * rstd; }
    }
}

__global__ __launch_bounds__(256)
void axpy_rows_kernel(float* __restrict__ acc, const float* __restrict__ v, int first, size_t n4) {
    for (size_t i = blockIdx.x * (size_t)blockDim.x + threadIdx.x; i < n4; i += (size_t)gridDim.x * blockDim.x) {
// ... 43 lines not shown
```

### uncertainty-vit_amd/csrc/rowwise.h

```cpp
#pragma once
#include <type_traits>
#include "common.h"

#define ROW_MAXV 8

template <class F>
static inline void dispatch_nv(int C, F&& f) {
    const int nv = (C + 255) / 256;
    if (nv <= 1) f(std::integral_constant<int, 1>{}); else if (nv == 2) f(std::integral_constant<int, 2>{});
    else if (nv == 3) f(std::integral_constant<int, 3>{}); else if (nv == 4) f(std::integral_constant<int, 4>{});
    else if (nv == 5) f(std::integral_constant<int, 5>{}); else f(std::integral_constant<int, ROW_MAXV>{});
}

template <int NV> struct RowVec { float4 v[NV]; };

template <int NV>
__device__ __forceinline__ void load_row(RowVec<NV>& r, const float* x, int C, int lane) {
    const int nv = C >> 2;
#pragma unroll
    for (int k = 0; k < NV; ++k) {
        const int i = lane + 64 * k;
        r.v[k] = i < nv ? ((const float4*)x)[i] : make_float4(0.f, 0.f, 0.f, 0.f);
    }
}

template <int NV>
__device__ __forceinline__ void row_stats(const RowVec<NV>& r, int C, int lane, float eps, float& mean, float& rstd) {
    const int nv = C >> 2;
    float s = 0.f;
#pragma unroll
    for (int k = 0; k < NV; ++k) s += r.v[k].x + r.v[k].y + r.v[k].z + r.v[k].w;
    mean = wave_sum(s) / C;
    float q = 0.f;
#pragma unroll
    for (int k = 0; k < NV; ++k) {
        if (lane + 64 * k < nv) {
            const float a = r.v[k].x - mean, b = r.v[k].y - mean, c = r.v[k].z - mean, d = r.v[k].w - mean;
            q += a * a + b * b + c * c + d * d;
        }
    }
    rstd = rsqrtf(wave_sum(q) / C + eps);
}

__device__ __forceinline__ float4 normalize4(const float4& v, float mean, float rstd) {
    return make_float4((v.x - mean) * rstd, (v.y - mean) * rstd, (v.z - mean) * rstd, (v.w - mean) * rstd);
}

template <int NV>
__device__ __forceinline__ void normalize_store(const RowVec<NV>& r, float mean, float rstd, const float* w, const float* b, bf16* y,
                                                int nv, int lane) {
#pragma unroll
    for (int k = 0; k < NV; ++k) {
        const int i = lane + 64 * k;
        if (i < nv) {
            const float4 h = normalize4(r.v[k], mean, rstd), ww = ((const float4*)w)[i], bb = ((const float4*)b)[i];
            ((bf16x4*)y)[i] = bf16x4{f2bf(h.x * ww.x + bb.x), f2bf(h.y * ww.y + bb.y), f2bf(h.z * ww.z + bb.z), f2bf(h.w * ww.w + bb.w)};
        }
    }
}
template <int NV>
__device__ __forceinline__ void normalize_store(const RowVec<NV>& r, float mean, float rstd, float* dst, bool accumulate, int nv, int lane) {
#pragma unroll
    for (int k = 0; k < NV; ++k) {
        const int i = lane + 64 * k;
        if (i < nv) {
            float4 o = normalize4(r.v[k], mean, rstd);
            if (accumulate) { const float4 a = ((const float4*)dst)[i]; o.x += a.x; o.y += a.y; o.z += a.z; o.w += a.w; }
            ((float4*)dst)[i] = o;
        }
    }
}

__device__ __forceinline__ bf16x4 bf16x4_zero() { return bf16x4{f2bf(0.f), f2bf(0.f), f2bf(0.f), f2bf(0.f)}; }

template <int NV>
__device__ __forceinline__ void store_zero_row(bf16* y, int nv, int lane) {
#pragma unroll
    for (int k = 0; k < NV; ++k)
        if (lane + 64 * k < nv) ((bf16x4*)y)[lane + 64 * k] = bf16x4_zero();
}

__device__ __forceinline__ void ls_apply(const float4& d, float dp, const bf16x4& y, const float4& gamma, bf16x4* dy, float4& ag, float4& ab) {
    const float e0 = d.x * dp, e1 = d.y * dp, e2 = d.z * dp, e3 = d.w * dp;
    ag.x += e0 * bf2f(y[0]); ag.y += e1 * bf2f(y[1]); ag.z += e2 * bf2f(y[2]); ag.w += e3 * bf2f(y[3]);
    const bf16x4 o = {f2bf(e0 * gamma.x), f2bf(e1 * gamma.y), f2bf(e2 * gamma.z), f2bf(e3 * gamma.w)};
    *dy = o;
    ab.x += bf2f(o[0]); ab.y += bf2f(o[1]); ab.z += bf2f(o[2]); ab.w += bf2f(o[3]);
}
```

### uncertainty-vit_amd/csrc/uvit_internal.h

```cpp
#pragma once
#include <hip/hip_runtime.h>
#include <stdint.h>
#include "common.h"

enum { EPI_BF16 = 0, EPI_QKV = 1, EPI_GELU = 2, EPI_RESID = 3, EPI_F32 = 4, EPI_PATCH = 5, EPI_DGELU = 6, EPI_QKV_ELU = 7,
       EPI_GELU_DG = 8,
       EPI_MULAUX = 9 };

struct GemmEpi {
    void* out = nullptr;
    void* out2 = nullptr;
    const float* bias = nullptr;
    const float* bias2 = nullptr;
    const float* gamma = nullptr;
    const float* resid = nullptr;
    const float* rowscale = nullptr;
    const void* aux = nullptr;
    const int64_t* mask = nullptr;
    const float* mask_token = nullptr;
    int ldo = 0;
    int tokens = 1;
    int patches = 1;
    int row0 = 0;
    int ngroup = 0;
// ... 45 lines not shown
                               int head_dim = 64);
int uvit_attn_dbias_reduce_launch(const void* ds_ws, float* dbias_slab, int accumulate, int B, int H, int N, int NP, hipStream_t s);

int uvit_attn2_fwd_launch(const void* qkv_m, const void* qkv_c, const float* biasP, void* out_m, void* out_c, float* lse,
                          int B, int H, int N, int NP, float scale, float p_drop, uint32_t seed, uint32_t layer, hipStream_t s);
size_t uvit_attn2_bwd_ws_bytes(int B, int H, int N);
int uvit_attn2_bwd_launch(const void* qkv_m, const void* qkv_c, const void* o_m, const void* o_c, const void* d_m, const void* d_c,
                          const float* biasP, const float* lse, float* delta, void* dqkv_m, void* dqkv_c, void* ds_ws, int want_ds,
                          int B, int H, int N, int NP, float scale, float p_drop, uint32_t seed, uint32_t layer, hipStream_t s);
int uvit_attn2_dbias_reduce_launch(const void* ds_ws, float* dbias_slab, int accumulate, int B, int H, int N, int NP, hipStream_t s);

struct LnFwd {
    const float* x = nullptr;
    const float* w = nullptr;
    const float* b = nullptr;
    bf16* y = nullptr;
    float* mean = nullptr;
    float* rstd = nullptr;
    int M = 0, C = 0;
    float eps = 0.f;
    const int* rowidx = nullptr;
    const int* count = nullptr;
    const int* pos = nullptr;
    float* xcopy = nullptr;
    int tokens = 0;
};
int uvit_ln_fwd_launch(const LnFwd& p, hipStream_t s);

struct LsNext {
    const bf16* y = nullptr;
    const float* gamma = nullptr;
    const float* rowscale = nullptr;
    bf16* dy = nullptr;
    float* dgamma = nullptr;
    float* dbias = nullptr;
    int tokens = 0;
    const int* pos = nullptr;
    const int* cnt = nullptr;
    int pad_base = 0;
    bf16* pad2 = nullptr;
    int pad2_cols = 0;
};
struct LnBwd {
    const bf16* dy = nullptr;
    const float* x = nullptr;
    const float* mean = nullptr;
    const float* rstd = nullptr;
    const float* w = nullptr;
    const float* dres = nullptr;
    float* dx = nullptr;
    float* dw = nullptr;
    float* db = nullptr;
    int M = 0, C = 0;
    int nrep = 1;
    size_t rep_stride = 0;
    const int* rowidx = nullptr;
    const int* count = nullptr;
    const int* pos = nullptr;
    LsNext next;
};
int uvit_ln_bwd_launch(const LnBwd& p, hipStream_t s);
int uvit_reduce_replicas_launch(const float* rep, float* out, size_t n, int nrep, size_t stride, hipStream_t s);
int uvit_target_accum_launch(const float* x, const int* rowidx, const int* count, float* acc, int first, int Mmax,
                             int C, float eps, hipStream_t s, const float* sub = nullptr,
                             int ln = 1);
int uvit_variance_loss_launch(const float* out, const int* count, float w, float margin, float loss_scale, float* scratch,
                              float* loss, float* std_loss0_out, void* dout_bf16, int Mmax, int C, hipStream_t s);
int uvit_gather_patch_rows_launch(const float* x, const float* sub, float* v, int B, int P, int C, hipStream_t s);
int uvit_colnorm_launch(float* v, int groups, int rows, int C, float eps, hipStream_t s);
int uvit_axpy_rows_launch(float* acc, const float* v, int first, size_t n, hipStream_t s);
int uvit_gather_masked_rows_launch(const float* dense, const int* rowidx, const int* count, float* out, int Mmax, int P, int C,
                                   hipStream_t s);
int uvit_target_finalize_launch(float* acc, const int* count, int n_layers, int post_ln, int Mmax, int C, float eps,
                                hipStream_t s);

int uvit_im2col_launch(const float* img, void* cols_bf16, int B, int Cin, int img_size, int patch, hipStream_t s);
int uvit_mask_compact_launch(const int64_t* mask, int* rowidx, int* count, int B, int P, hipStream_t s);
int uvit_set_cls_launch(float* x, const float* cls, const float* pos, int B, int N, int C, hipStream_t s);
int uvit_relpos_gather_launch(const float* table, const int* index, float* biasP, int H, int N, int NP, hipStream_t s);
int uvit_relpos_scatter_launch(const float* slab, int nslab, const int* index, float* dtable, int H, int N, int NP,
                               hipStream_t s);
int uvit_ls_bwd_launch(const float* dx, const LsNext& ls, int M, int C, int nrep, size_t rep_stride, hipStream_t s,
                       const int* rowidx = nullptr, const int* count = nullptr);
int uvit_rows_guard_launch(const int* count, int limit, float* loss, hipStream_t s);
int uvit_colsum_launch(const void* y_bf16, int ld, int col0, int ncols, int M, float* out, int nrep, size_t rep_stride,
                       hipStream_t s);
int uvit_smooth_l1_launch(const float* out, const float* target, const int* count, float beta, int l2, float loss_scale,
                          float* loss, void* dout_bf16, int Mmax, int C, hipStream_t s);
int uvit_token_bwd_launch(const float* dx, const int64_t* mask, void* dpatch_bf16, float* dcls, float* dmask_token,
                          int B, int P, int C, hipStream_t s);
int uvit_transpose_batch_launch(const void* descs_dev, int ndesc, int max_tiles, hipStream_t s);
int uvit_droppath_launch(float* scales, const float* rates_dev, int depth, int nbr, int B, uint32_t seed, uint32_t step,
                         hipStream_t s);
int uvit_droppath_lists_launch(const float* scales, int* pos, int* bmap, int* rows, int* cnt, int nlists, int B, int tokens,
                               int rows_stride, const int* host_counts, hipStream_t s);
int uvit_droppath_lists_guard_launch(const int* cnt, int nlists, float* loss, hipStream_t s);
int uvit_add_pos_launch(float* x, const float* pos, int B, int N, int C, hipStream_t s);
int uvit_pos_bwd_launch(const float* dx, float* dpos, int B, int N, int C, hipStream_t s);
int uvit_synth_batch_launch(float* images, int64_t* mask, int B, int chans, int img_size, int patches, int n_mask, uint32_t seed,
                            uint32_t it, hipStream_t s);
int uvit_poison_if_nonfinite_launch(const float* loss, float* dst, int* sticky, hipStream_t s);
int uvit_wasserstein_loss_launch(const float* out_m, const float* out_c, const float* tgt_m, const float* tgt_c, const int* count,
                                 float lam, float loss_scale, float* scratch, float* loss, void* dout_m_bf16, void* dout_c_bf16,
                                 int Mmax, int C, hipStream_t s);

int uvit_ema_launch(float* ema, const float* p, void* ema_bf16, size_t n, float decay, hipStream_t s, const float* guard_loss = nullptr,
                    const double* guard_sumsq = nullptr);
int uvit_sumsq_launch(const float* g, size_t n, double* out, hipStream_t s);
int uvit_adamw_launch(float* p, const float* g, float* m, float* v, void* p_bf16, size_t n, size_t n_decay, float lr,
                      float wd, float b1, float b2, float eps, int step, const double* sumsq, float max_norm,
                      float grad_scale, float* gnorm_out, hipStream_t s, const float* guard_loss = nullptr,
                      float* ema = nullptr, void* ema_bf16 = nullptr, float ema_decay = 0.f,
                      int* sticky_poison = nullptr,
                      const float* sched_dev = nullptr, int sched_len = 0, int sched_idx = 0);
int uvit_zero_launch(void* dst, size_t bytes, hipStream_t s);
int uvit_cast_bf16_launch(const float* src, void* dst_bf16, size_t n, hipStream_t s);

struct TransposeDesc { const void* src; void* dst; int rows; int cols; int tile0; int pad; };
```

### uncertainty-vit_amd/native.py

```python
import ctypes as C
import os
import subprocess

import torch

_HERE = os.path.dirname(os.path.abspath(__file__))
LIB_PATH = os.path.join(_HERE, "libuvit.so")
MAX_DEPTH = 64


class UvitError(RuntimeError):
    pass


_ERR = {-1: "bad argument", -2: "unsupported shape", -3: "HIP launch/runtime error", -4: "workspace too small"}


def check(rc, what=""):
    if rc != 0:
        raise UvitError(f"libuvit: {what} failed: {_ERR.get(rc, rc)} ({rc})")


class Config(C.Structure):
    _fields_ = [(n, C.c_int32) for n in ("img_size", "patch_size", "in_chans", "embed_dim", "depth", "num_heads",
                                          "mlp_hidden", "use_shared_rel_pos_bias", "use_abs_pos_emb", "batch")] + \
               [("ln_eps", C.c_float), ("attn_drop_rate", C.c_float), ("drop_path_rate", C.c_float),
                ("bias_chunk", C.c_int32), ("two_stream", C.c_int32)]


class LayoutEntry(C.Structure):
    _fields_ = [("name", C.c_char * 96), ("offset", C.c_int64), ("numel", C.c_int64), ("ndim", C.c_int32),
                ("decay", C.c_int32), ("shape", C.c_int64 * 4)]


class Buffers(C.Structure):
    _fields_ = [(n, C.c_void_p) for n in ("params", "grads", "adam_m", "adam_v", "ema", "params_bf16",
                                           "params_bf16_t", "ema_bf16", "rel_index", "workspace")] + \
               [("workspace_bytes", C.c_int64)]


class StepParams(C.Structure):
    _fields_ = [("target_layers", C.c_int32 * MAX_DEPTH), ("n_target_layers", C.c_int32),
                ("target_layer_norm_last", C.c_int32), ("post_target_layer_norm", C.c_int32), ("l2_loss", C.c_int32),
                ("l1_beta", C.c_float), ("loss_scale", C.c_float), ("clip_grad", C.c_float), ("lr", C.c_float),
                ("weight_decay", C.c_float), ("beta1", C.c_float), ("beta2", C.c_float), ("eps", C.c_float),
                ("opt_step", C.c_int32), ("ema_decay", C.c_float), ("do_ema", C.c_int32), ("grad_scale", C.c_float),
                ("seed", C.c_uint32), ("it", C.c_uint32), ("train_dropout", C.c_int32), ("lambda_pretraining", C.c_float),
                ("sched_dev", C.c_void_p), ("sched_len", C.c_int32), ("sched_index", C.c_int32),
                ("layer_results_fc", C.c_int32), ("var_w0", C.c_float), ("var_margin0", C.c_float),
                ("target_batch_norm", C.c_int32), ("target_instance_norm", C.c_int32), ("post_target_instance_norm", C.c_int32),
                ("n_rows_hint", C.c_int32)]


class WgradProblem(C.Structure):
    _fields_ = [("Y", C.c_void_p), ("X", C.c_void_p), ("C", C.c_void_p), ("bias", C.c_void_p), ("bias2", C.c_void_p),
                ("bias_end", C.c_int32), ("bias2_begin", C.c_int32), ("M", C.c_int32), ("N", C.c_int32), ("K", C.c_int32),
                ("ldy", C.c_int32), ("ldx", C.c_int32), ("ldc", C.c_int32)]


class GemmEpilogue(C.Structure):
    _fields_ = [(n, C.c_void_p) for n in ("out", "out2", "bias", "bias2", "gamma", "resid", "rowscale", "aux", "mask",
                                           "mask_token")] + [("ldo", C.c_int32), ("tokens", C.c_int32), ("patches", C.c_int32),
                                                             ("row0", C.c_int32)]


class Tuning(C.Structure):
    _fields_ = [("nt_variant", C.c_int32), ("tn_variant", C.c_int32), ("tn_split_target", C.c_int32),
                ("wgrad_group_chunks", C.c_int32), ("nt_group", C.c_int32), ("nt_persist", C.c_int32)]

    @classmethod
    def default(cls, **over):
        t = cls()
        lib().uvit_tuning_default(C.byref(t))
        for k, v in over.items():
            setattr(t, k, v)
        return t


class GemmNtPlanInfo(C.Structure):
    _fields_ = [("kernel", C.c_int32), ("rows", C.c_int32), ("grid", C.c_int32), ("tail_rows", C.c_int32)]


class LsRider(C.Structure):
    _fields_ = [(n, C.c_void_p) for n in ("y", "gamma", "rowscale", "dy", "dgamma", "dbias")] + \
               [("tokens", C.c_int32), ("pos", C.c_void_p), ("cnt", C.c_void_p), ("pad_base", C.c_int32), ("pad2", C.c_void_p),
                ("pad2_cols", C.c_int32)]


class WgradSplit(C.Structure):
    _fields_ = [("bias_s1", C.c_void_p), ("bias2_s1", C.c_void_p), ("s1_row", C.c_int32)]


class TransposeDesc(C.Structure):
    _fields_ = [("src", C.c_void_p), ("dst", C.c_void_p), ("rows", C.c_int32), ("cols", C.c_int32), ("tile0", C.c_int32),
                ("pad", C.c_int32)]


class AugmentDesc(C.Structure):
    _fields_ = [("offset", C.c_int64)] + \
               [(n, C.c_int32) for n in ("h", "w", "flip", "crop_x", "crop_y", "crop_w", "crop_h", "resize_w", "resize_h", "win_x",
                                          "win_y", "filter", "n_jitter")] + \
               [("jitter_op", C.c_int32 * 3), ("jitter_factor", C.c_float * 3), ("reserved", C.c_int32)]


_vp, _i, _i64, _f, _u32 = C.c_void_p, C.c_int, C.c_int64, C.c_float, C.c_uint32
_PROTOTYPES = {
    "uvit_version": (_i, []),
    "uvit_source_hash": (C.c_char_p, []),
    "uvit_layout_count": (_i, [_vp]),
    "uvit_layout_get": (_i, [_vp, _i, _vp]),
    "uvit_arena_numel": (_i64, [_vp, _vp]),
    "uvit_workspace_bytes": (_i64, [_vp]),
    "uvit_engine_create": (_vp, [_vp, _vp, _vp, _vp]),
    "uvit_engine_destroy": (None, [_vp]),
    "uvit_engine_sync_shadows": (_i, [_vp, _i, _vp]),
    "uvit_engine_forward_features": (_i, [_vp, _i, _vp, _vp, _i, _i, _u32, _u32, _vp]),
    "uvit_engine_forward_tail": (_i, [_vp, _i, _i, _i, _i, _u32, _u32, _vp]),
    "uvit_engine_head": (_i, [_vp, _i, _i, _vp, _vp, _vp]),
    "uvit_engine_ws_ptr": (_vp, [_vp, C.c_char_p, _i]),
    "uvit_engine_compact_rows": (_i, [_vp]),
    "uvit_step_begin": (_i, [_vp, _vp, _vp, _vp, _vp]),
    "uvit_step_backward_layer": (_i, [_vp, _i, _vp, _vp]),
    "uvit_step_backward_embed": (_i, [_vp, _vp]),
    "uvit_step_wait_layer_grads": (_i, [_vp, _i, _vp]),
    "uvit_step_update": (_i, [_vp, _vp, _vp]),
    "uvit_train_step": (_i, [_vp, _vp, _vp, _vp, _vp]),
    "uvit_engine_read_stats": (_i, [_vp, _vp, _vp]),
    "uvit_engine_read_stats_async": (_i, [_vp, _vp, _vp]),
    "uvit_tuning_default": (None, [_vp]),
    "uvit_engine_set_tuning": (_i, [_vp, _vp]),
    "uvit_op_wgrad_group": (_i, [_vp, _i, _vp, _vp]),
    "uvit_engine_set_streams": (_i, [_vp, _i]),
    "uvit_engine_set_drop_path_rows": (_i, [_vp, _i]),
    "uvit_drop_path_kept_counts": (_i, [_i, _f, _i, _i, _u32, _u32, _vp]),
    "uvit_engine_profile": (_i, [_vp, _i, _i]),
    "uvit_engine_profile_read": (_i, [_vp, _vp, _vp, _vp]),
    "uvit_engine_profile_read_kind": (_i, [_vp, _i, _vp, _vp, _vp, _vp]),
    "uvit_op_gemm_nt": (_i, [_i, _vp, _vp, _i, _i, _i, _i, _i, _vp, _vp]),
    "uvit_op_gemm_nt_tuned": (_i, [_i, _vp, _vp, _i, _i, _i, _i, _i, _vp, _vp, _vp, _vp]),
    "uvit_op_gemm_nt_plan": (_i, [_i, _i, _i, _i, _i, _i, _i, _i, _vp, _i, _vp]),
    "uvit_op_gemm_nt_sched": (_i, [_i, _vp, _vp, _i, _i, _i, _i, _i, _vp, _vp, _vp, _vp]),
    "uvit_op_gemm_tn": (_i, [_vp, _vp, _i, _i, _i, _i, _i, _vp, _i, _vp, _vp]),
    "uvit_op_wasserstein_loss": (_i, [_vp, _vp, _vp, _vp, _vp, _f, _f, _vp, _vp, _vp, _vp, _i, _i, _vp]),
    "uvit_op_attn_fwd": (_i, [_vp, _vp, _vp, _vp, _i, _i, _i, _i, _f, _f, _u32, _u32, _vp]),
    "uvit_op_attn_bwd_ws_bytes": (_i64, [_i, _i, _i]),
    "uvit_op_attn_bwd": (_i, [_vp, _vp, _vp, _vp, _vp, _vp, _vp, _vp, _i, _vp, _i, _i, _i, _i, _f, _f, _u32, _u32, _vp]),
    "uvit_op_attn_fwd_hd": (_i, [_vp, _vp, _vp, _vp, _i, _i, _i, _i, _i, _f, _f, _u32, _u32, _vp]),
    "uvit_op_attn_bwd_hd": (_i, [_vp, _vp, _vp, _vp, _vp, _vp, _vp, _vp, _i, _vp, _i, _i, _i, _i, _i, _f, _f, _u32, _u32, _vp]),
    "uvit_op_attn2_fwd": (_i, [_vp, _vp, _vp, _vp, _vp, _vp, _i, _i, _i, _i, _f, _f, _u32, _u32, _vp]),
    "uvit_op_attn2_bwd_ws_bytes": (_i64, [_i, _i, _i]),
    "uvit_op_attn2_bwd": (_i, [_vp] * 12 + [_i, _vp, _i, _i, _i, _i, _f, _f, _u32, _u32, _vp]),
    "uvit_op_relpos_gather": (_i, [_vp, _vp, _vp, _i, _i, _i, _vp]),
    "uvit_op_relpos_scatter": (_i, [_vp, _i, _vp, _vp, _i, _i, _i, _vp]),
    "uvit_op_ln_fwd": (_i, [_vp, _vp, _vp, _vp, _vp, _vp, _i, _i, _f, _vp]),
    "uvit_op_ln_bwd": (_i, [_vp, _vp, _vp, _vp, _vp, _vp, _vp, _vp, _vp, _i, _i, _vp]),
    "uvit_op_ln_fwd_walk": (_i, [_vp, _vp, _vp, _vp, _vp, _vp, _i, _i, _f, _vp, _vp, _vp, _vp, _i, _vp]),
    "uvit_op_ln_bwd_walk": (_i, [_vp] * 9 + [_i, _i, _i, _i64, _vp, _vp, _vp, _vp, _vp]),
    "uvit_op_ls_bwd": (_i, [_vp, _vp, _i, _i, _i, _i64, _vp, _vp, _vp]),
    "uvit_op_colsum": (_i, [_vp, _i, _i, _i, _i, _vp, _i, _i64, _vp]),
    "uvit_op_reduce_replicas": (_i, [_vp, _vp, _i64, _i, _i64, _vp]),
    "uvit_op_droppath_lists": (_i, [_vp, _vp, _vp, _vp, _vp, _i, _i, _i, _i, _vp, _vp]),
    "uvit_op_gemm_nt_rows": (_i, [_i, _vp, _vp, _i, _i, _i, _i, _i, _vp, _vp, _vp, _vp, _vp]),
    "uvit_op_wgrad_group_split": (_i, [_vp, _vp, _i, _vp, _vp]),
    "uvit_op_token_bwd": (_i, [_vp, _vp, _vp, _vp, _vp, _i, _i, _i, _vp]),
    "uvit_op_transpose_batch": (_i, [_vp, _i, _i, _vp]),
    "uvit_op_ema": (_i, [_vp, _vp, _vp, _i64, _f, _vp]),
    "uvit_op_sumsq": (_i, [_vp, _i64, _vp, _vp]),
    "uvit_op_adamw": (_i, [_vp, _vp, _vp, _vp, _vp, _i64, _i64, _f, _f, _f, _f, _f, _i, _vp, _f, _f, _vp, _vp]),
    "uvit_op_smooth_l1": (_i, [_vp, _vp, _vp, _f, _i, _f, _vp, _vp, _i, _i, _vp]),
    "uvit_op_target_accum": (_i, [_vp, _vp, _vp, _vp, _i, _i, _i, _f, _vp]),
    "uvit_op_variance_loss": (_i, [_vp, _vp, _f, _f, _f, _vp, _vp, _vp, _vp, _i, _i, _vp]),
    "uvit_op_target_finalize": (_i, [_vp, _vp, _i, _i, _i, _i, _f, _vp]),
    "uvit_op_mask_compact": (_i, [_vp, _vp, _vp, _i, _i, _vp]),
    "uvit_op_im2col": (_i, [_vp, _vp, _i, _i, _i, _i, _vp]),
    "uvit_op_synth_batch": (_i, [_vp, _vp, _i, _i, _i, _i, _i, _u32, _u32, _vp]),
    "uvit_op_droppath": (_i, [_vp, _vp, _i, _i, _u32, _u32, _vp]),
    "uvit_op_cast_bf16": (_i, [_vp, _vp, _i64, _vp]),
    "uvit_op_augment_ws_bytes": (_i64, [_vp, _i, _i]),
    "uvit_op_augment_batch": (_i, [_vp, _i64, _vp, _i, _i, _vp, _vp, _vp, _vp, _i64, _vp]),
    "uvit_op_probe_pool_ws_bytes": (_i64, [_i, _i, _i]),
    "uvit_op_probe_pool_norm": (_i, [_vp, _vp, _vp, _i, _i, _i, _f, _vp]),
    "uvit_op_probe_logits": (_i, [_vp, _vp, _vp, _vp, _i, _i, _i, _vp]),
    "uvit_op_probe_ce": (_i, [_vp, _vp, _f, _vp, _vp, _vp, _vp, _i, _i, _vp]),
    "uvit_op_probe_head_grad": (_i, [_vp, _vp, _vp, _vp, _i, _i, _i, _vp]),
    "uvit_op_calib_softmax": (_i, [_vp, _vp, _i, _i, _vp]),
    "uvit_op_calib_confidence": (_i, [_vp, _vp, _vp, _i, _i, _vp, _vp, _vp, _vp, _vp, _i, _i, _vp]),
    "uvit_op_calib_tace": (_i, [_vp, _vp, C.c_double, _i, _i, _vp, _vp, _i, _i, _vp]),
    "uvit_op_calib_auroc": (_i, [_vp, _vp, _vp, _vp, _i, _i, _vp]),
    "uvit_op_stability_ranks": (_i, [_vp, _vp, _i, _i, _vp]),
    "uvit_op_stability_sequences": (_i, [_vp, _vp, _i, _i, _i, _i, _vp]),
    "uvit_op_gp_features": (_i, [_vp] * 5 + [_f, _f] + [_vp] * 3 + [_i, _i, _i, _vp]),
    "uvit_op_gp_precision_update": (_i, [_vp, _vp, _i, _i, C.c_double, _vp]),
    "uvit_op_gp_ln_grad_ws_bytes": (_i64, [_i, _i, _i]),
    "uvit_op_gp_ln_grad": (_i, [_vp] * 5 + [_f] + [_vp] * 3 + [_i, _i, _i, _i, _vp]),
    "uvit_op_gp_variance": (_i, [_vp, _vp, C.c_double, _vp, _i, _i, _vp]),
    "uvit_op_gp_mean_field": (_i, [_vp, _vp, C.c_double, _vp, _i, _i, _vp]),
    "uvit_op_het_noise": (_i, [_vp, _vp, _i, _i, _i, _i, _u32, _i, _vp]),
    "uvit_op_het_mc_ws_bytes": (_i64, [_i, _i, _i, _i]),
    "uvit_op_het_mc_forward": (_i, [_vp] * 5 + [_i, _i, _i, _i, _f, _f, _u32, _i, _vp]),
    "uvit_op_het_mc_backward": (_i, [_vp] * 5 + [_i, _i, _i, _i, _f, _f, _u32, _i, _vp]),
    "uvit_op_ens_bag_weights": (_i, [_vp, _i, _i, _u32, _vp]),
    "uvit_op_ens_ce": (_i, [_vp, _vp, _vp, _f, _vp, _vp, _vp, _vp, _i, _i, _i, _vp]),
    "uvit_op_ens_clip": (_i, [_vp, _vp, _i, _i, _i, _f, _vp]),
    "uvit_op_ens_combine": (_i, [_vp, _i, _vp, _vp, _i, _i, _i, _vp]),
    "uvit_op_detect_rows": (_i, [_vp, _vp, _vp, _i64, _i64, _vp, _i, _i, _vp]),
    "uvit_op_detect_column": (_i, [_vp, _i, _i64, _vp, _i, _vp]),
    "uvit_op_detect_ws_bytes": (_i64, [_i, _i]),
    "uvit_op_detect_metrics": (_i, [_vp, _i64, _vp, _i, _i, _vp, _vp, _vp, _i64, _vp]),
    "uvit_op_ts_ws_bytes": (_i64, [_i, _i]),
    "uvit_op_ts_fit": (_i, [_vp, _i64, _vp, _i, _i, C.c_double, C.c_double, C.c_double, _i, _vp, _vp, _i64, _vp]),
    "uvit_op_ts_scale": (_i, [_vp, _vp, _i64, _i64, _vp, _i, _i, _vp]),
    "uvit_op_cp_scores": (_i, [_vp, _i64, _vp, _vp, _i, _i, _i, C.c_double, _i, _vp, _vp]),
    "uvit_op_cp_ws_bytes": (_i64, [_i, _i]),
    "uvit_op_cp_quantile": (_i, [_vp, _i, _vp, _i, _vp, _vp, _i64, _vp]),
    "uvit_op_cp_counter_count": (_i64, [_i, _i]),
    "uvit_op_cp_sets": (_i, [_vp, _i64, _vp, _vp, _i, _i, _i, C.c_double, _i, _vp, _i, _vp, _vp, _vp, _i64, _vp]),
    "uvit_op_cp_finish": (_i, [_vp, _vp, _i, _i, _vp]),
    "uvit_op_lap_factors_ws_bytes": (_i64, [_i, _i, _i]),
    "uvit_op_lap_factors": (_i, [_vp, _vp, _i64, _vp, _vp, _vp, _vp, _vp, _i64, _i, _i, _i, _vp]),
    "uvit_op_lap_prepare": (_i, [_vp, _vp, _vp, C.c_double, _vp, _i, _i, _vp]),
    "uvit_op_lap_variance_ws_bytes": (_i64, [_i, _i, _i]),
    "uvit_op_lap_variance": (_i, [_vp, _vp, _vp, _vp, _vp, _i64, _i, _i, _i, _vp]),
    "uvit_op_lap_probit": (_i, [_vp, _i64, _vp, C.c_double, _vp, _i64, _vp, _i, _i, _vp]),
    "uvit_op_maha_accumulate_ws_bytes": (_i64, [_i, _i, _i]),
    "uvit_op_maha_accumulate": (_i, [_vp] * 8 + [_i64, _i, _i, _i, _vp]),
    "uvit_op_maha_scores_ws_bytes": (_i64, [_i, _i, _i]),
    "uvit_op_maha_scores": (_i, [_vp] * 10 + [_i64, _vp, _vp, _vp, _i64, _i, _i, _i, _vp]),
    "uvit_op_knn_rows": (_i, [_vp] * 5 + [_i, _i, _i, _vp]),
    "uvit_op_knn_search_ws_bytes": (_i64, [_i, _i, _i, _i, _i]),
    "uvit_op_knn_search": (_i, [_vp] * 6 + [_i64, _vp, _i64, _i, _i, _i, _i, _i, _vp]),
    "uvit_op_knn_scores": (_i, [_vp, _vp, _i64, _vp, _i, _vp, _vp, _vp, _i64, _vp, _vp, _i, _i, _i, C.c_double, _vp]),
    "uvit_op_vim_scores_ws_bytes": (_i64, [_i, _i, _i, _i]),
    "uvit_op_vim_scores": (_i, [_vp, _vp, _vp, C.c_double] + [_vp] * 7 + [_i64, _i, _i, _i, _i, _vp]),
    "uvit_op_mcd_state_bytes": (_i64, [_i, _i]),
    "uvit_op_mcd_accumulate": (_i, [_vp, _vp, _i, _i, _i, _vp]),
    "uvit_op_mcd_finalize": (_i, [_vp, _i, _i, _vp, _vp, _i, _i, _vp]),
}
SYMBOLS = list(_PROTOTYPES)

_lib = None

# ... 74 lines not shown
```

Before: 5413.

## Derive layer-scale gamma gradient from weight gradients instead of saving branch outputs

Stops saving the proj and fc2 branch outputs (projout/mlpout) in the forward pass by default. The layer-scale dgamma is instead reconstructed algebraically as (sum over W·dW rows + bias·dbias)/gamma in a new small kernel that runs after wgrad on the weight stream. This removes a bf16 activation write in forward and a read in the LN/LS backward kernels, adding a per-channel dot-product pass over the weights. It risks numerical error when gamma is near zero (returns 0 there) and relies on the dW buffers being complete before the kernel runs. The old path stays available via an environment variable.

Result: no change. 5443, median of 2 (+0.6%).

```diff
diff --git a/include/uvit.h b/include/uvit.h
--- a/include/uvit.h
+++ b/include/uvit.h
@@ -181,6 +181,11 @@
                         const int32_t* count, const int32_t* pos, const uvit_ls_rider* next, uvit_stream stream);
 int uvit_op_ls_bwd(const float* dx, const uvit_ls_rider* rider, int M, int C, int nrep, int64_t rep_stride, const int32_t* rowidx,
                    const int32_t* count, uvit_stream stream);
+typedef struct uvit_ls_dgamma_term {
+    const void* W_bf16; const float* dW; const float* bias; const float* dbias; int32_t K; int32_t ldw; int32_t lddw;
+} uvit_ls_dgamma_term;
+int uvit_op_ls_dgamma_from_wgrad(const uvit_ls_dgamma_term* terms, int nterms, const float* gamma, float* out, int C, int nrep,
+                                 int64_t rep_stride, uvit_stream stream);
 int uvit_op_colsum(const void* y_bf16, int ld, int col0, int ncols, int M, float* out, int nrep, int64_t rep_stride, uvit_stream stream);
 int uvit_op_reduce_replicas(const float* rep, float* out, int64_t n, int nrep, int64_t stride, uvit_stream stream);
 int uvit_op_droppath_lists(const float* scales, int32_t* pos, int32_t* bmap, int32_t* rows, int32_t* cnt, int nlists, int B, int tokens,
diff --git a/uncertainty-vit_amd/csrc/elementwise.hip b/uncertainty-vit_amd/csrc/elementwise.hip
--- a/uncertainty-vit_amd/csrc/elementwise.hip
+++ b/uncertainty-vit_amd/csrc/elementwise.hip
@@ -106,7 +106,7 @@
     }
 }
 
-template <int NV>
+template <int NV, bool WITH_Y>
 __global__ __launch_bounds__(256)
 void ls_bwd_kernel(const float* __restrict__ dx, const bf16* __restrict__ y, const float* __restrict__ gamma,
                    const float* __restrict__ rowscale, bf16* __restrict__ dy, float* __restrict__ dgamma,
@@ -130,13 +130,62 @@
             if (i < nv) {
                 const float4 d = ((const float4*)(dx + (size_t)xr * C))[i];
                 const float4 g = ((const float4*)gamma)[i];
-                const bf16x4 yy = ((const bf16x4*)(y + (size_t)xr * C))[i];
-                ls_apply(d, dp, yy, g, (bf16x4*)(dy + (size_t)row * C) + i, ag[k], ab[k]);
+                if constexpr (WITH_Y) {
+                    const bf16x4 yy = ((const bf16x4*)(y + (size_t)xr * C))[i];
+                    ls_apply(d, dp, yy, g, (bf16x4*)(dy + (size_t)row * C) + i, ag[k], ab[k]);
+                } else {
+                    ls_apply(d, dp, g, (bf16x4*)(dy + (size_t)row * C) + i, ab[k]);
+                }
             }
         }
     }
-    block_col_atomic(ag, dgamma, nv, red);
+    if constexpr (WITH_Y) block_col_atomic(ag, dgamma, nv, red);
     block_col_atomic(ab, dbias, nv, red);
+}
+
+#define LSDG_WAVES 4
+#define LSDG_DEPTH 6
+__global__ __launch_bounds__(LSDG_WAVES * 64)
+void ls_dgamma_from_wgrad_kernel(LsDgammaList list) {
+    const LsDgamma& p = list.v[blockIdx.y];
+    const int lane = threadIdx.x & 63;
+    const int c = blockIdx.x * LSDG_WAVES + (threadIdx.x >> 6);
+    if (c >= p.C) return;
+    float acc = 0.f;
+    for (int t = 0; t < p.nterms; ++t) {
+        const LsDgammaTerm& q = p.term[t];
+        const bf16* w = q.W + (size_t)c * q.ldw;
+        const float* d = q.dW + (size_t)c * q.lddw;
+        for (int k0 = lane * 8; k0 < q.K; k0 += 512 * LSDG_DEPTH) {
+            bf16x8 wv[LSDG_DEPTH];
+            float4 d0[LSDG_DEPTH], d1[LSDG_DEPTH];
+#pragma unroll
+            for (int u = 0; u < LSDG_DEPTH; ++u) {
+                const int k = k0 + 512 * u;
+                if (k < q.K) { wv[u] = *(const bf16x8*)(w + k); d0[u] = *(const float4*)(d + k); d1[u] = *(const float4*)(d + k + 4); }
+            }
+#pragma unroll
+            for (int u = 0; u < LSDG_DEPTH; ++u) {
+                if (k0 + 512 * u < q.K) {
+                    acc += bf2f(wv[u][0]) * d0[u].x; acc += bf2f(wv[u][1]) * d0[u].y; acc += bf2f(wv[u][2]) * d0[u].z; acc += bf2f(wv[u][3]) * d0[u].w;
+                    acc += bf2f(wv[u][4]) * d1[u].x; acc += bf2f(wv[u][5]) * d1[u].y; acc += bf2f(wv[u][6]) * d1[u].z; acc += bf2f(wv[u][7]) * d1[u].w;
+                }
+            }
+        }
+    }
+    acc = wave_sum(acc);
+    for (int t = 0; t < p.nterms; ++t) {
+        const LsDgammaTerm& q = p.term[t];
+        float db = 0.f;
+        for (int r0 = 0; r0 < p.nrep; r0 += 64) {
+            const float v = r0 + lane < p.nrep ? q.db[(size_t)(r0 + lane) * p.rep_stride + c] : 0.f;
+            const int n = min(64, p.nrep - r0);
+            for (int j = 0; j < n; ++j) db += __shfl(v, j, 64);
+        }
+        acc += q.b[c] * db;
+    }
+    const float g = p.gamma[c];
+    if (lane == 0) p.out[c] = g != 0.f ? acc / g : 0.f;
 }
 
 #define CS_ROWS 256
@@ -375,9 +424,28 @@
                        const int* rowidx, const int* count) {
     if (C % 4 || C > ROW_MAXV * 256 || (rowidx && !count)) return UVIT_ERR_SHAPE;
     dispatch_nv(C, [&](auto nv) {
-        hipLaunchKernelGGL(ls_bwd_kernel<decltype(nv)::value>, dim3((M + CP_ROWS - 1) / CP_ROWS), dim3(256), 0, s, dx, ls.y, ls.gamma, ls.rowscale,
-                           ls.dy, ls.dgamma, ls.dbias, M, C, ls.tokens, nrep > 0 ? nrep : 1, rep_stride, rowidx, count);
+        constexpr int NV = decltype(nv)::value;
+        hipLaunchKernelGGL((ls.y ? ls_bwd_kernel<NV, true> : ls_bwd_kernel<NV, false>), dim3((M + CP_ROWS - 1) / CP_ROWS), dim3(256), 0, s, dx, ls.y,
+                           ls.gamma, ls.rowscale, ls.dy, ls.dgamma, ls.dbias, M, C, ls.tokens, nrep > 0 ? nrep : 1, rep_stride, rowidx, count);
     });
+    return uvit_check_launch();
+}
+int uvit_ls_dgamma_from_wgrad_launch(const LsDgamma* v, int n, hipStream_t s) {
+    if (!v || n < 1 || n > LSDG_VECS) return UVIT_ERR_SHAPE;
+    LsDgammaList list;
+    int maxC = 0;
+    for (int i = 0; i < n; ++i) {
+        const LsDgamma& p = v[i];
+        if (p.C < 1 || p.nterms < 1 || p.nterms > LSDG_TERMS || p.nrep < 1) return UVIT_ERR_SHAPE;
+        for (int t = 0; t < p.nterms; ++t) {
+            const LsDgammaTerm& q = p.term[t];
+            if (q.K < 8 || (q.K % 8) || q.ldw < q.K || (q.ldw % 8) || q.lddw < q.K || (q.lddw % 4)) return UVIT_ERR_SHAPE;
+            if (((uintptr_t)q.W | (uintptr_t)q.dW) & 15) return UVIT_ERR_SHAPE;
+        }
+        list.v[i] = p;
+        maxC = p.C > maxC ? p.C : maxC;
+    }
+    hipLaunchKernelGGL(ls_dgamma_from_wgrad_kernel, dim3((maxC + LSDG_WAVES - 1) / LSDG_WAVES, n), dim3(LSDG_WAVES * 64), 0, s, list);
     return uvit_check_launch();
 }
 __global__ void rows_guard_kernel(const int* __restrict__ count, int limit, float* __restrict__ loss) {
diff --git a/uncertainty-vit_amd/csrc/engine.hip b/uncertainty-vit_amd/csrc/engine.hip
--- a/uncertainty-vit_amd/csrc/engine.hip
+++ b/uncertainty-vit_amd/csrc/engine.hip
@@ -178,6 +178,10 @@
 };
 
 static size_t roundup(size_t x, size_t m) { return (x + m - 1) / m * m; }
+static bool ls_saved_y() {
+    static const bool on = getenv("UVIT_LS_SAVED_Y") && getenv("UVIT_LS_SAVED_Y")[0] == '1';
+    return on;
+}
 static std::vector<float> dp_rates_linspace(int depth, float rate);
 
 static void plan_workspace(uvit_engine* e, Bump& b) {
@@ -581,6 +585,7 @@
     const int Bc = p.Bc, M = Bc * e->N, C = e->C, Hd = e->Hd, S = e->S;
     const size_t Mp = e->Mpad;
     const bool save = p.kind == PASS_STUDENT;
+    const bool save_y = save && ls_saved_y();
     const BranchRows at = branch_rows(e, l, 0, p.rows, Bc), ml = branch_rows(e, l, 1, p.rows, Bc);
     LnFwd n1; n1.x = x_in; n1.w = w.f + o.n1w; n1.b = w.f + o.n1b; n1.y = a.ln1; n1.mean = a.mean1; n1.rstd = a.rstd1; n1.M = at.rows; n1.C = C;
     n1.eps = e->cfg.ln_eps;
@@ -606,7 +611,7 @@
     };
     auto prof_end = [&](bool on) { if (on) { (void)hipEventRecord(e->prof_ev[e->prof_used + 1], s); e->prof_used += 2; } };
     for (int st = 0; st < S; ++st) {
-        GemmEpi pj; pj.out = x_mid + st * Mp * C; pj.out2 = save ? a.projout + st * Mp * C : nullptr; pj.bias = w.f + o.projb[st];
+        GemmEpi pj; pj.out = x_mid + st * Mp * C; pj.out2 = save_y ? a.projout + st * Mp * C : nullptr; pj.bias = w.f + o.projb[st];
         pj.gamma = w.f + o.g1; pj.resid = x_in + st * Mp * C; pj.rowscale = dp_ptr(e, p.dp_on, l, st, 0, Bc); pj.ldo = C; pj.tokens = e->N;
         pj.rowmap = at.rowmap[st]; pj.rowcount = at.rowcnt[st];
         const bool pp = prof_begin(UVIT_PROF_PROJ, at.n[st]);
@@ -631,7 +636,7 @@
     CHECK(GEMM_NT(save ? EPI_GELU_DG : EPI_GELU, a.ln2, w.b + o.fc1w, ml.rows, Hd, C, C, C, &f1, s));
     prof_end(prof);
     for (int st = 0; st < S; ++st) {
-        GemmEpi f2; f2.out = x_out + st * Mp * C; f2.out2 = save ? a.mlpout + st * Mp * C : nullptr; f2.bias = w.f + o.fc2b;
+        GemmEpi f2; f2.out = x_out + st * Mp * C; f2.out2 = save_y ? a.mlpout + st * Mp * C : nullptr; f2.bias = w.f + o.fc2b;
         f2.gamma = w.f + o.g2; f2.resid = x_mid + st * Mp * C; f2.rowscale = dp_ptr(e, p.dp_on, l, st, 1, Bc); f2.ldo = C; f2.tokens = e->N;
         f2.rowmap = ml.rowmap[st]; f2.rowcount = ml.rowcnt[st];
         const bool pf2 = prof_begin(UVIT_PROF_FC2, ml.n[st]);
@@ -913,10 +918,11 @@
         qk.bias = RP(o.qb[0]); qk.bias_end = C; qk.bias2 = RP(o.vb[0]); qk.bias2_begin = 2 * C;
         if (S == 2) { qk.bias_s1 = RP(o.qb[1]); qk.bias2_s1 = RP(o.vb[1]); qk.s1_row = (int)Mp; }
     }
+    const bool with_y = ls_saved_y();
     auto mlp_rider = [&](int layer, int st, const BranchRows& br, bf16* dY) {
         const LayerOff& L = e->lo.L[layer];
-        LsNext n; n.y = e->acts[layer].mlpout + st * Mp * C; n.gamma = pf + L.g2; n.rowscale = dp_ptr(e, dp_on, layer, st, 1, e->B);
-        n.dy = dY + br.off[st] * C; n.dgamma = RP(L.g2); n.dbias = RP(L.fc2b); n.tokens = e->N;
+        LsNext n; if (with_y) n.y = e->acts[layer].mlpout + st * Mp * C; n.gamma = pf + L.g2; n.rowscale = dp_ptr(e, dp_on, layer, st, 1, e->B);
+        n.dy = dY + br.off[st] * C; if (with_y) n.dgamma = RP(L.g2); n.dbias = RP(L.fc2b); n.tokens = e->N;
         return n;
     };
     if (l == e->cfg.depth - 1)
@@ -933,8 +939,9 @@
         LnBwd b; b.dy = e->dLN + ml.off[st] * C; b.x = e->XM[l] + eo; b.mean = a.mean2 + ml.off[st]; b.rstd = a.rstd2 + ml.off[st]; b.w = pf + o.n2w;
         b.dres = e->dXa + eo; b.dx = e->dXb + eo; b.dw = RP(o.n2w); b.db = RP(o.n2b); b.C = C; b.nrep = NREP; b.rep_stride = e->n_nd;
         LsNext& n = b.next;
-        n.y = a.projout + eo; n.gamma = pf + o.g1; n.rowscale = dp_ptr(e, dp_on, l, st, 0, e->B); n.dy = dY2 + at.off[st] * C;
-        n.dgamma = RP(o.g1); n.dbias = RP(o.projb[st]); n.tokens = e->N; n.pos = at.d[st].pos;
+        if (with_y) { n.y = a.projout + eo; n.dgamma = RP(o.g1); }
+        n.gamma = pf + o.g1; n.rowscale = dp_ptr(e, dp_on, l, st, 0, e->B); n.dy = dY2 + at.off[st] * C;
+        n.dbias = RP(o.projb[st]); n.tokens = e->N; n.pos = at.d[st].pos;
         if (ln2_samples) { b.M = M; b.pos = ml.d[st].pos; n.cnt = at.d[st].cnt; if (at.mode == ROWS_LIST) { n.pad2 = dqkv; n.pad2_cols = 3 * C; } }
         else { b.M = ml.n[st]; b.rowidx = ml.rowmap[st]; b.count = ml.rowcnt[st]; }
         CHECK(uvit_ln_bwd_launch(b, s));
@@ -966,6 +973,19 @@
     e->slab_started = true;
     if (e->dual) { HIPCHECK(hipEventRecord(e->ev_x, s)); HIPCHECK(hipStreamWaitEvent(ws, e->ev_x, 0)); }
     CHECK(wgrad(e, wg, nwg, ws));
+    if (!with_y) {
+        const bf16* wb = (const bf16*)e->buf.params_bf16;
+        LsDgamma gv[2];
+        LsDgamma& g1 = gv[0]; g1.gamma = pf + o.g1; g1.out = RP(o.g1); g1.C = C; g1.nrep = NREP; g1.rep_stride = e->n_nd; g1.nterms = S;
+        for (int st = 0; st < S; ++st) {
+            LsDgammaTerm& t = g1.term[st];
+            t.W = wb + o.projw[st]; t.dW = g + o.projw[st]; t.b = pf + o.projb[st]; t.db = RP(o.projb[st]); t.K = C; t.ldw = C; t.lddw = C;
+        }
+        LsDgamma& g2 = gv[1]; g2.gamma = pf + o.g2; g2.out = RP(o.g2); g2.C = C; g2.nrep = NREP; g2.rep_stride = e->n_nd; g2.nterms = 1;
+        LsDgammaTerm& t = g2.term[0];
+        t.W = wb + o.fc2w; t.dW = g + o.fc2w; t.b = pf + o.fc2b; t.db = RP(o.fc2b); t.K = Hd; t.ldw = Hd; t.lddw = Hd;
+        CHECK(uvit_ls_dgamma_from_wgrad_launch(gv, 2, ws));
+    }
     if (e->dual) HIPCHECK(hipEventRecord(e->ev_wdone[l], ws));
     GemmEpi d4; d4.out = e->dLN; d4.ldo = C;
     CHECK(GEMM_NT(EPI_BF16, dqkv, wt + o.qkvw, at.rows, C, 3 * C, 3 * C, 3 * C, &d4, s));
@@ -1218,6 +1238,18 @@
     if (M <= 0 || C <= 0 || r->tokens <= 0) return UVIT_ERR_SHAPE;
     return uvit_ls_bwd_launch(dx, ls_from_abi(r), M, C, nrep, (size_t)rep_stride, S(st), rowidx, count);
 }
+extern "C" int uvit_op_ls_dgamma_from_wgrad(const uvit_ls_dgamma_term* terms, int nterms, const float* gamma, float* out, int C, int nrep,
+                                            int64_t rep_stride, uvit_stream st) {
+    if (!terms || !gamma || !out || nterms < 1 || nterms > LSDG_TERMS || nrep < 1 || rep_stride < 0) return UVIT_ERR_ARG;
+    LsDgamma p; p.gamma = gamma; p.out = out; p.C = C; p.nrep = nrep; p.rep_stride = (size_t)rep_stride; p.nterms = nterms;
+    for (int t = 0; t < nterms; ++t) {
+        const uvit_ls_dgamma_term& q = terms[t];
+        if (!q.W_bf16 || !q.dW || !q.bias || !q.dbias) return UVIT_ERR_ARG;
+        LsDgammaTerm& d = p.term[t];
+        d.W = (const bf16*)q.W_bf16; d.dW = q.dW; d.b = q.bias; d.db = q.dbias; d.K = q.K; d.ldw = q.ldw; d.lddw = q.lddw;
+    }
+    return uvit_ls_dgamma_from_wgrad_launch(&p, 1, S(st));
+}
 extern "C" int uvit_op_colsum(const void* y, int ld, int col0, int ncols, int M, float* out, int nrep, int64_t rep_stride, uvit_stream st) {
     if (!y || !out || nrep < 1 || rep_stride < 0) return UVIT_ERR_ARG;
     if (M <= 0 || ncols <= 0 || col0 < 0 || col0 + ncols > ld) return UVIT_ERR_SHAPE;
diff --git a/uncertainty-vit_amd/csrc/norm.hip b/uncertainty-vit_amd/csrc/norm.hip
--- a/uncertainty-vit_amd/csrc/norm.hip
+++ b/uncertainty-vit_amd/csrc/norm.hip
@@ -5,6 +5,7 @@
 #define LN_WAVES 4
 
 enum LnWalk { WALK_ROWS, WALK_SAMPLES };
+enum LsMode { LS_NONE = 0, LS_Y = 1, LS_NOY = 2 };
 
 template <int NV, LnWalk WALK>
 __global__ __launch_bounds__(LN_WAVES * 64)
@@ -40,17 +41,17 @@
 
 #define LNB_WAVES 8
 
-template <int NV, bool LS>
+template <int NV, LsMode LS>
 struct LnbRow {
     float4 x[NV], dres[NV];
-    bf16x4 dy[NV], y[LS ? NV : 1];
+    bf16x4 dy[NV], y[LS == LS_Y ? NV : 1];
     float mean, rstd, dp;
     int xr;
     int ar;
     int yr;
 };
 
-template <int NV, LnWalk WALK, bool LS>
+template <int NV, LnWalk WALK, LsMode LS>
 __device__ __forceinline__ void lnb_load(LnbRow<NV, LS>& r, int row, const bf16* dy, const float* x, const int* map,
                                          const float* mean_i, const float* rstd_i, const float* dres, const LsNext& ls,
                                          int C, int nv, int lane) {
@@ -83,7 +84,7 @@
                 r.dy[k] = ((const bf16x4*)(dy + (size_t)r.ar * C))[i];
             }
             r.dres[k] = WALK == WALK_SAMPLES || dres ? ((const float4*)(dres + (size_t)r.xr * C))[i] : make_float4(0.f, 0.f, 0.f, 0.f);
-            if constexpr (LS) if (WALK == WALK_ROWS || r.yr >= 0) r.y[k] = ((const bf16x4*)(ls.y + (size_t)r.xr * C))[i];
+            if constexpr (LS == LS_Y) if (WALK == WALK_ROWS || r.yr >= 0) r.y[k] = ((const bf16x4*)(ls.y + (size_t)r.xr * C))[i];
         }
     }
 }
@@ -97,7 +98,7 @@
     }
 }
 
-template <int NV, LnWalk WALK, bool LS>
+template <int NV, LnWalk WALK, LsMode LS>
 __global__ __launch_bounds__(LNB_WAVES * 64)
 void ln_bwd_kernel(const bf16* __restrict__ dy, const float* __restrict__ x, const int* __restrict__ map ,
                    const int* __restrict__ count, const float* __restrict__ mean_i, const float* __restrict__ rstd_i,
@@ -112,7 +113,8 @@
     if constexpr (WALK == WALK_SAMPLES && LS) { if (ls.cnt && blockIdx.x == gridDim.x - 1) lnb_pad_fill<NV>(ls, C, nv, lane, wave); }
     float4 ww[NV], gm[LS ? NV : 1];
     RowVec<NV> aw, ab;
-    RowVec<LS ? NV : 1> ag, ay;
+    RowVec<LS == LS_Y ? NV : 1> ag;
+    RowVec<LS ? NV : 1> ay;
 #pragma unroll
     for (int k = 0; k < NV; ++k) {
         aw.v[k] = make_float4(0.f, 0.f, 0.f, 0.f); ab.v[k] = aw.v[k];
@@ -120,7 +122,8 @@
     }
 #pragma unroll
     for (int k = 0; k < (LS ? NV : 1); ++k) {
-        ag.v[k] = make_float4(0.f, 0.f, 0.f, 0.f); ay.v[k] = ag.v[k]; gm[k] = ag.v[k];
+        ay.v[k] = make_float4(0.f, 0.f, 0.f, 0.f); gm[k] = ay.v[k];
+        if constexpr (LS == LS_Y) ag.v[k] = ay.v[k];
         if constexpr (LS) { if (lane + 64 * k < nv) gm[k] = ((const float4*)ls.gamma)[lane + 64 * k]; }
     }
     const int row_end = min((int)(blockIdx.x + 1) * rows_per_block, n_valid);
@@ -160,8 +163,10 @@
                 if (own) o = make_float4(o.x + rstd * (g[k].x - s1 - h[k].x * s2), o.y + rstd * (g[k].y - s1 - h[k].y * s2),
                                          o.z + rstd * (g[k].z - s1 - h[k].z * s2), o.w + rstd * (g[k].w - s1 - h[k].w * s2));
                 ((float4*)(dx + (size_t)cur.xr * C))[i] = o;
-                if constexpr (LS) if (cur.yr >= 0)
+                if constexpr (LS == LS_Y) if (cur.yr >= 0)
                     ls_apply(o, cur.dp, cur.y[k], gm[k], (bf16x4*)(ls.dy + (size_t)cur.yr * C) + i, ag.v[k], ay.v[k]);
+                if constexpr (LS == LS_NOY) if (cur.yr >= 0)
+                    ls_apply(o, cur.dp, gm[k], (bf16x4*)(ls.dy + (size_t)cur.yr * C) + i, ay.v[k]);
             }
         }
         if (more) cur = nxt;
@@ -185,7 +190,8 @@
         if (64 * k < nv) {
             fold(aw.v[k], dw, k);
             fold(ab.v[k], db, k);
-            if constexpr (LS) { fold(ag.v[k], ls.dgamma, k); fold(ay.v[k], ls.dbias, k); }
+            if constexpr (LS == LS_Y) fold(ag.v[k], ls.dgamma, k);
+            if constexpr (LS) fold(ay.v[k], ls.dbias, k);
         }
     }
 }
@@ -273,8 +279,8 @@
     const int rpb = lnb_rows(p.M, LNB_BLOCKS_PER_CU);
     dispatch_nv(p.C, [&](auto nv) {
         constexpr int NV = decltype(nv)::value;
-        auto kernel = samples ? (ls ? ln_bwd_kernel<NV, WALK_SAMPLES, true> : ln_bwd_kernel<NV, WALK_SAMPLES, false>)
-                              : (ls ? ln_bwd_kernel<NV, WALK_ROWS, true> : ln_bwd_kernel<NV, WALK_ROWS, false>);
+        auto kernel = samples ? (!ls ? ln_bwd_kernel<NV, WALK_SAMPLES, LS_NONE> : n.y ? ln_bwd_kernel<NV, WALK_SAMPLES, LS_Y> : ln_bwd_kernel<NV, WALK_SAMPLES, LS_NOY>)
+                              : (!ls ? ln_bwd_kernel<NV, WALK_ROWS, LS_NONE> : n.y ? ln_bwd_kernel<NV, WALK_ROWS, LS_Y> : ln_bwd_kernel<NV, WALK_ROWS, LS_NOY>);
         hipLaunchKernelGGL(kernel, dim3((p.M + rpb - 1) / rpb), dim3(LNB_WAVES * 64), 0, s, p.dy, p.x, samples ? p.pos : p.rowidx, p.count,
                            p.mean, p.rstd, p.w, p.dres, p.dx, p.dw, p.db, p.M, p.C, p.nrep > 0 ? p.nrep : 1, p.rep_stride, n, rpb);
     });
diff --git a/uncertainty-vit_amd/csrc/rowwise.h b/uncertainty-vit_amd/csrc/rowwise.h
--- a/uncertainty-vit_amd/csrc/rowwise.h
+++ b/uncertainty-vit_amd/csrc/rowwise.h
@@ -87,3 +87,9 @@
     *dy = o;
     ab.x += bf2f(o[0]); ab.y += bf2f(o[1]); ab.z += bf2f(o[2]); ab.w += bf2f(o[3]);
 }
+__device__ __forceinline__ void ls_apply(const float4& d, float dp, const float4& gamma, bf16x4* dy, float4& ab) {
+    const float e0 = d.x * dp, e1 = d.y * dp, e2 = d.z * dp, e3 = d.w * dp;
+    const bf16x4 o = {f2bf(e0 * gamma.x), f2bf(e1 * gamma.y), f2bf(e2 * gamma.z), f2bf(e3 * gamma.w)};
+    *dy = o;
+    ab.x += bf2f(o[0]); ab.y += bf2f(o[1]); ab.z += bf2f(o[2]); ab.w += bf2f(o[3]);
+}
diff --git a/uncertainty-vit_amd/csrc/uvit_internal.h b/uncertainty-vit_amd/csrc/uvit_internal.h
--- a/uncertainty-vit_amd/csrc/uvit_internal.h
+++ b/uncertainty-vit_amd/csrc/uvit_internal.h
@@ -151,6 +151,25 @@
                                hipStream_t s);
 int uvit_ls_bwd_launch(const float* dx, const LsNext& ls, int M, int C, int nrep, size_t rep_stride, hipStream_t s,
                        const int* rowidx = nullptr, const int* count = nullptr);
+#define LSDG_TERMS 2
+struct LsDgammaTerm {
+    const bf16* W = nullptr;
+    const float* dW = nullptr;
+    const float* b = nullptr;
+    const float* db = nullptr;
+    int K = 0, ldw = 0, lddw = 0;
+};
+struct LsDgamma {
+    LsDgammaTerm term[LSDG_TERMS];
+    int nterms = 0;
+    const float* gamma = nullptr;
+    float* out = nullptr;
+    int C = 0, nrep = 1;
+    size_t rep_stride = 0;
+};
+#define LSDG_VECS 2
+struct LsDgammaList { LsDgamma v[LSDG_VECS]; };
+int uvit_ls_dgamma_from_wgrad_launch(const LsDgamma* v, int n, hipStream_t s);
 int uvit_rows_guard_launch(const int* count, int limit, float* loss, hipStream_t s);
 int uvit_colsum_launch(const void* y_bf16, int ld, int col0, int ncols, int M, float* out, int nrep, size_t rep_stride,
                        hipStream_t s);
diff --git a/uncertainty-vit_amd/native.py b/uncertainty-vit_amd/native.py
--- a/uncertainty-vit_amd/native.py
+++ b/uncertainty-vit_amd/native.py
@@ -85,6 +85,11 @@
     _fields_ = [(n, C.c_void_p) for n in ("y", "gamma", "rowscale", "dy", "dgamma", "dbias")] + \
                [("tokens", C.c_int32), ("pos", C.c_void_p), ("cnt", C.c_void_p), ("pad_base", C.c_int32), ("pad2", C.c_void_p),
                 ("pad2_cols", C.c_int32)]
+
+
+class LsDgammaTerm(C.Structure):
+    _fields_ = [("W", C.c_void_p), ("dW", C.c_void_p), ("bias", C.c_void_p), ("dbias", C.c_void_p), ("K", C.c_int32),
+                ("ldw", C.c_int32), ("lddw", C.c_int32)]
 
 
 class WgradSplit(C.Structure):
@@ -157,6 +162,7 @@
     "uvit_op_ln_fwd_walk": (_i, [_vp, _vp, _vp, _vp, _vp, _vp, _i, _i, _f, _vp, _vp, _vp, _vp, _i, _vp]),
     "uvit_op_ln_bwd_walk": (_i, [_vp] * 9 + [_i, _i, _i, _i64, _vp, _vp, _vp, _vp, _vp]),
     "uvit_op_ls_bwd": (_i, [_vp, _vp, _i, _i, _i, _i64, _vp, _vp, _vp]),
+    "uvit_op_ls_dgamma_from_wgrad": (_i, [_vp, _i, _vp, _vp, _i, _i, _i64, _vp]),
     "uvit_op_colsum": (_i, [_vp, _i, _i, _i, _i, _vp, _i, _i64, _vp]),
     "uvit_op_reduce_replicas": (_i, [_vp, _vp, _i64, _i, _i64, _vp]),
     "uvit_op_droppath_lists": (_i, [_vp, _vp, _vp, _vp, _vp, _i, _i, _i, _i, _vp, _vp]),
```
